# google-research/frame-interpolation

Hardware: NVIDIA H100
Metric: interpolated_frames_per_sec_1080p (higher is better)
Workload: dtype f16x2-split (activations/weights as fp16 hi+lo planes; fp32 accumulate)

## Files before the change

### frame_interpolation_b200/csrc/film_common.cuh

```cuda
#pragma once
#include <cuda_bf16.h>
#include <cuda_fp16.h>
#include <cuda_runtime.h>
#include <stdint.h>

namespace film {

#ifdef FILM_SPLIT_FP16
typedef __half sp_t;
#define FILM_SPLIT_NAME "fp16x2"
#else
typedef __nv_bfloat16 sp_t;
#define FILM_SPLIT_NAME "bf16x2"
#endif

constexpr float kLeaky = 0.2f;

struct ActView {
  sp_t* hi;
  sp_t* lo;
  int B, H, W, C;
};

__device__ __forceinline__ float sp_to_float(sp_t v) {
#ifdef FILM_SPLIT_FP16
  return __half2float(v);
#else
  return __bfloat162float(v);
#endif
}
__device__ __forceinline__ sp_t float_to_sp(float v) {
#ifdef FILM_SPLIT_FP16
  return __float2half_rn(v);
#else
  return __float2bfloat16_rn(v);
#endif
}

__device__ __forceinline__ void split2(float x, sp_t& hi, sp_t& lo) {
  hi = float_to_sp(x);
  lo = float_to_sp(x - sp_to_float(hi));
}

#ifndef FILM_SPLIT_FP16
__device__ __forceinline__ void split_pack2(float a, float b, uint32_t& hi, uint32_t& lo) {
  const __nv_bfloat162 h2 = __floats2bfloat162_rn(a, b);
  hi = *reinterpret_cast<const uint32_t*>(&h2);
  const float ra = a - __uint_as_float(hi << 16);
  const float rb = b - __uint_as_float(hi & 0xffff0000u);
  const __nv_bfloat162 l2 = __floats2bfloat162_rn(ra, rb);
  lo = *reinterpret_cast<const uint32_t*>(&l2);
}
__device__ __forceinline__ void split_pack2_generic(float a, float b, uint32_t& hi, uint32_t& lo) {
#else
__device__ __forceinline__ void split_pack2(float a, float b, uint32_t& hi, uint32_t& lo) {
  asm("cvt.rn.satfinite.f16x2.f32 %0, %1, %2;" : "=r"(hi) : "f"(b), "f"(a));
  const float2 hf = __half22float2(*reinterpret_cast<const __half2*>(&hi));
  asm("cvt.rn.satfinite.f16x2.f32 %0, %1, %2;" : "=r"(lo) : "f"(b - hf.y), "f"(a - hf.x));
}
__device__ __forceinline__ void split_pack2_generic(float a, float b, uint32_t& hi, uint32_t& lo) {
#endif
  sp_t ah, al, bh, bl;
  split2(a, ah, al);
  split2(b, bh, bl);
  hi = (uint32_t)(*reinterpret_cast<unsigned short*>(&ah)) |
       ((uint32_t)(*reinterpret_cast<unsigned short*>(&bh)) << 16);
  lo = (uint32_t)(*reinterpret_cast<unsigned short*>(&al)) |
       ((uint32_t)(*reinterpret_cast<unsigned short*>(&bl)) << 16);
}

__device__ __forceinline__ float sp_bits_to_float(uint32_t bits16) {
#ifdef FILM_SPLIT_FP16
  unsigned short s = (unsigned short)bits16;
  return __half2float(*reinterpret_cast<__half*>(&s));
#else
  return __uint_as_float(bits16 << 16);
#endif
}

__device__ __forceinline__ void unpack8(const uint4& h, const uint4& l, float* v) {
  const uint32_t hw[4] = {h.x, h.y, h.z, h.w};
  const uint32_t lw[4] = {l.x, l.y, l.z, l.w};
#pragma unroll
  for (int i = 0; i < 4; ++i) {
#ifndef FILM_SPLIT_FP16
    v[2 * i] = __uint_as_float(hw[i] << 16) + __uint_as_float(lw[i] << 16);
    v[2 * i + 1] = __uint_as_float(hw[i] & 0xffff0000u) + __uint_as_float(lw[i] & 0xffff0000u);
#else
    const float2 hf = __half22float2(*reinterpret_cast<const __half2*>(&hw[i]));
    const float2 lf = __half22float2(*reinterpret_cast<const __half2*>(&lw[i]));
    v[2 * i] = hf.x + lf.x;
    v[2 * i + 1] = hf.y + lf.y;
#endif
  }
}

__device__ __forceinline__ void pack8(const float* v, uint4& h, uint4& l) {
  split_pack2(v[0], v[1], h.x, l.x);
  split_pack2(v[2], v[3], h.y, l.y);
  split_pack2(v[4], v[5], h.z, l.z);
  split_pack2(v[6], v[7], h.w, l.w);
}

__device__ __forceinline__ void st256(void* p, const uint4& a, const uint4& b) {
  uint4* q = reinterpret_cast<uint4*>(p);
  q[0] = a;
  q[1] = b;
}
__device__ __forceinline__ void ld256_nc(const void* p, uint4& a, uint4& b) {
  const uint4* q = reinterpret_cast<const uint4*>(p);
  a = __ldg(q);
  b = __ldg(q + 1);
}
__device__ __forceinline__ void pack_store16(const float* v, sp_t* hi_dst, sp_t* lo_dst) {
  uint4 h0, l0, h1, l1;
  pack8(v, h0, l0);
  pack8(v + 8, h1, l1);
  st256(hi_dst, h0, h1);
  st256(lo_dst, l0, l1);
}
__device__ __forceinline__ uint32_t pack2_hi(float a, float b) {
#ifdef FILM_SPLIT_FP16
  uint32_t hi;
  asm("cvt.rn.satfinite.f16x2.f32 %0, %1, %2;" : "=r"(hi) : "f"(b), "f"(a));
  return hi;
#else
  const __nv_bfloat162 h2 = __floats2bfloat162_rn(a, b);
  return *reinterpret_cast<const uint32_t*>(&h2);
#endif
}
__device__ __forceinline__ void pack_store16_hi(const float* v, sp_t* hi_dst) {
  uint4 h0, h1;
  h0.x = pack2_hi(v[0], v[1]);   h0.y = pack2_hi(v[2], v[3]);   h0.z = pack2_hi(v[4], v[5]);   h0.w = pack2_hi(v[6], v[7]);
  h1.x = pack2_hi(v[8], v[9]);   h1.y = pack2_hi(v[10], v[11]); h1.z = pack2_hi(v[12], v[13]); h1.w = pack2_hi(v[14], v[15]);
  st256(hi_dst, h0, h1);
}
__device__ __forceinline__ void unpack8_hi(const uint4& h, float* v) {
  const uint32_t hw[4] = {h.x, h.y, h.z, h.w};
#pragma unroll
  for (int i = 0; i < 4; ++i) {
#ifndef FILM_SPLIT_FP16
    v[2 * i] = __uint_as_float(hw[i] << 16);
    v[2 * i + 1] = __uint_as_float(hw[i] & 0xffff0000u);
#else
    const float2 hf = __half22float2(*reinterpret_cast<const __half2*>(&hw[i]));
    v[2 * i] = hf.x;
    v[2 * i + 1] = hf.y;
#endif
  }
}
__device__ __forceinline__ void load_unpack16_hi(const sp_t* hi_src, float* v) {
  uint4 h0, h1;
  ld256_nc(hi_src, h0, h1);
  unpack8_hi(h0, v);
  unpack8_hi(h1, v + 8);
}
__device__ __forceinline__ void load_unpack16(const sp_t* hi_src, const sp_t* lo_src, float* v) {
  uint4 h0, h1, l0, l1;
  ld256_nc(hi_src, h0, h1);
  ld256_nc(lo_src, l0, l1);
  unpack8(h0, l0, v);
  unpack8(h1, l1, v + 8);
}

__device__ __forceinline__ float leaky(float x) { return x >= 0.f ? x : x * kLeaky; }

}
```

### frame_interpolation_b200/csrc/film_conv3x3_tc.cu

```cuda
#include <cuda.h>
#include <cuda_runtime.h>
#include <stdint.h>

#include <type_traits>

#include "film_conv.h"
#include "film_tc_ptx.cuh"

namespace film {
namespace {
using namespace tc;

constexpr int kConsumers = 256;
constexpr int kThreads = kConsumers + 128;
__host__ __device__ constexpr int a_plane_bytes(int kc, int th, int tw) { return (th + 2) * tw * kc * 2; }
__host__ __device__ constexpr int a_stage_bytes(int kc, int th, int tw) { return 2 * a_plane_bytes(kc, th, tw); }
constexpr int kHaloW = 10;
__host__ __device__ constexpr int halo_box_bytes(int kc, int th) { return (th + 2) * kHaloW * kc * 2; }
__host__ __device__ constexpr int halo_plane_bytes(int kc, int th) { return (halo_box_bytes(kc, th) + 1023) & ~1023; }
__host__ __device__ constexpr int a_stage_bytes_h(int kc, int th, int tw, int halo, int planes = 2) {
  return planes * (halo ? halo_plane_bytes(kc, th) : a_plane_bytes(kc, th, tw));
}
constexpr int kMaxRing = 8;
constexpr int kSmemLimit = 227 * 1024;
constexpr int kBarBytes = 8 * (4 * kMaxRing + 4);
constexpr int kFixedBytes = kBarBytes + 16 + 512 * 4  + 64  + 1024  + 64;
constexpr int kHeadW3 = 64 * 32 * 4, kHeadMisc = 512;
constexpr int kHeadBytes = kHeadW3 + kHeadMisc;
constexpr int kPxnStageWg = 64 * 64 * 2;
constexpr int kPxnStageBytes = 2 * kPxnStageWg;
inline int epi_scratch_bytes(int epi_mode, int pxn) { return epi_mode == 3 ? kHeadBytes : pxn ? kPxnStageBytes : 0; }

__host__ __device__ inline int w_tap_bytes(int bn, int kc, int planes = 2) { return bn * kc * 2 * planes; }

template <int BN, int KC, bool kPartial, bool kHalo, bool kOne, bool kRes, bool kPxN = false>
__global__ void __launch_bounds__(kThreads, 1) k_conv3x3_tc(const ConvProblem* __restrict__ prob) {
  static_assert(!kPxN || (BN == 64 && KC == 64), "pixels on N: Cout = 64 (one M = 64 weight tile), 64-channel chunks");
  extern __shared__ uint8_t smem_raw[];
  constexpr bool one = kOne;
  const int planes = one ? 1 : 2;
  constexpr int kWPlane = BN * KC * 2;
  const int kWTap = kWPlane * planes;
  const int kTileH = prob->tile_h, kTileW = prob->tile_w;
  constexpr int kHaloTileH = kPxN ? 32 : 16;
  constexpr int kHaloBox = halo_box_bytes(KC, kHaloTileH), kHaloPlane = halo_plane_bytes(KC, kHaloTileH);
  constexpr bool halo = kHalo;
  const int kAPlane = halo ? kHaloPlane : a_plane_bytes(KC, kTileH, kTileW);
  const int kAStage = planes * kAPlane;
  const int kRowStep = kTileW * KC * 2;
  constexpr bool kFused = BN <= 128 && !kPxN;
  constexpr int kAccRegs = kPxN ? 64 : (kFused ? 2 * BN : BN) / 2;
  constexpr int kWgPx = kPxN ? 128 : 64;

  const int NA = prob->v2_na, NW = prob->v2_nw;
  const bool resident = prob->v2_resident != 0;
  const int nsrc = prob->nsrc;
  const int tiles_x = prob->tiles_x, tiles_per_img = prob->tiles_y * prob->tiles_x;
  const int cout = prob->cout;
  const int n_nt = (cout + BN - 1) / BN;
  const int ntiles = prob->B * tiles_per_img * n_nt;
  constexpr int kStageTaps = kHalo ? 9 : 3;
  constexpr bool kPacked = kPartial && kPxN;
  const int part_lo = prob->v2_part_lo, part_hi = prob->v2_part_hi;
  int nab = 0;
  for (int s = 0; s < nsrc; ++s) nab += prob->src[s].nchunk * (kHalo ? 1 : 3);
  const int nkb = nab * kStageTaps - (kPacked ? (part_hi - part_lo) * (kStageTaps - kStageTaps / 3) : 0);

  const FastDiv div_nt(n_nt, ntiles), div_img(tiles_per_img, ntiles), div_tx(tiles_x, ntiles);
  const bool pair = prob->pair != 0;
  const int rank = pair ? (int)cluster_ctarank() : 0;
  const int nsp = prob->B * tiles_per_img;
  const int nwork = pair ? ((nsp + 1) / 2) * n_nt : ntiles;
  const int w_first = pair ? (int)blockIdx.x >> 1 : (int)blockIdx.x, w_step = pair ? (int)gridDim.x >> 1 : (int)gridDim.x;
  auto decode = [&](int work, int& sp, int& nti) {
    div_nt.divmod(work, sp, nti);
    if (pair) sp = 2 * sp + rank;
  };

  const uint32_t raw = smem_u32(smem_raw);
  const uint32_t base = (raw + 1023u) & ~1023u;
  uint8_t* gen_base = smem_raw + (base - raw);
  const uint32_t a_base = base;
  const uint32_t w_base = a_base + (uint32_t)NA * kAStage;
  const uint32_t w_bytes = resident ? (uint32_t)nkb * kWTap : (uint32_t)NW * kWTap;
  const uint32_t tail = w_base + w_bytes;
  const uint32_t tail_off = (uint32_t)NA * kAStage + w_bytes;
  float* bias_smem = reinterpret_cast<float*>(gen_base + tail_off + kBarBytes + 16);
  int* src_tab = reinterpret_cast<int*>(gen_base + tail_off + kBarBytes + 16 + 512 * 4);

  const int warp = threadIdx.x >> 5, lane = threadIdx.x & 31;

  if (warp == 8 && lane == 0) {
    for (int s = 0; s < kMaxRing; ++s) {
      mbar_init(tail + 8u * s, 1);
      mbar_init(tail + 8u * (kMaxRing + s), 2);
      mbar_init(tail + 8u * (2 * kMaxRing + s), 1);
      mbar_init(tail + 8u * (3 * kMaxRing + s), pair ? 4 : 2);
    }
    for (int s = 0; s < kMaxSrc; ++s) {
      src_tab[2 * s] = s < nsrc ? prob->src[s].nchunk : 0;
      src_tab[2 * s + 1] = s < nsrc ? prob->src[s].c_off : 0;
      src_tab[2 * kMaxSrc + s] = s < nsrc ? prob->src[s].bswap : 0;
    }
    asm volatile("fence.mbarrier_init.release.cluster;" ::: "memory");
  }
  if (warp < 8)
    for (int i = threadIdx.x; i < n_nt * BN; i += kConsumers) bias_smem[i] = (i < cout) ? prob->bias[i] : 0.f;
  __syncthreads();
  if (pair) cluster_sync_all();
  auto leave = [&]() {
    if (pair) cluster_sync_all();
  };

  if (warp >= 8) {
    regs_dec<40>();
    if (warp > 8) {
      leave();
      return;
    }
    const CUtensorMap* tm_w_hi = &prob->tm_w_hi;
    const CUtensorMap* tm_w_lo = &prob->tm_w_lo;
    if (resident && elect_one()) {
      mbar_expect_tx(tail + 8u * (2 * kMaxRing), (uint32_t)nkb * kWTap);
      for (int kb = 0; kb < nkb; ++kb) {
        tma_load_2d(w_base + kb * kWTap, tm_w_hi, tail + 8u * (2 * kMaxRing), kb * KC, 0);
        if (!one) tma_load_2d(w_base + kb * kWTap + kWPlane, tm_w_lo, tail + 8u * (2 * kMaxRing), kb * KC, 0);
      }
    }
    __syncwarp();
    RingPos ra, rw;
    for (int tile = w_first; tile < nwork; tile += w_step) {
      int sp, nti, b, rem, ty, tx;
      decode(tile, sp, nti);
      div_img.divmod(sp, b, rem);
      div_tx.divmod(rem, ty, tx);
      const int n0 = nti * BN, y0 = ty * kTileH, x0 = tx * kTileW;
      {
        const int nt = tile + w_step;
        int next_sp, nnt;
        decode(nt < nwork ? nt : 0, next_sp, nnt);
        if (nt < nwork && next_sp != sp && next_sp < nsp && elect_one()) {
          int nb, nrem, nty, ntx;
          div_img.divmod(next_sp, nb, nrem);
          div_tx.divmod(nrem, nty, ntx);
          const int ny0 = nty * kTileH, nx0 = ntx * kTileW;
          for (int s = 0; s < nsrc; ++s)
            for (int ch = 0; ch < src_tab[2 * s]; ++ch) {
              const int cc = src_tab[2 * s + 1] + ch * KC;
              tma_prefetch_4d(&prob->tm_a_hi[s], cc, nx0 - 1, ny0 - 1, nb);
              if (!one) tma_prefetch_4d(&prob->tm_a_lo[s], cc, nx0 - 1, ny0 - 1, nb);
              if (!halo) {
                tma_prefetch_4d(&prob->tm_a_hi[s], cc, nx0 + 1, ny0 - 1, nb);
                if (!one) tma_prefetch_4d(&prob->tm_a_lo[s], cc, nx0 + 1, ny0 - 1, nb);
              }
            }
        }
        __syncwarp();
      }
      int kb = 0, ab = 0;
      for (int s = 0; s < nsrc; ++s) {
        const int nchunk = src_tab[2 * s], c_off = src_tab[2 * s + 1];
        const int bs = src_tab[2 * kMaxSrc + s] ? prob->B - 1 - b : b;
        const CUtensorMap* tm_hi = &prob->tm_a_hi[s];
        const CUtensorMap* tm_lo = &prob->tm_a_lo[s];
        for (int ch = 0; ch < nchunk; ++ch) {
          const int nst = halo ? 1 : 3;
          for (int dx = 0; dx < nst; ++dx, ++ab) {
            const int st = ra.stage;
            mbar_wait(tail + 8u * (kMaxRing + st), ra.phase ^ 1u);
            if (elect_one()) {
              const uint32_t sa = a_base + st * kAStage, bar = tail + 8u * st;
              mbar_expect_tx(bar, halo ? (uint32_t)(planes * kHaloBox) : (uint32_t)kAStage);
              tma_load_4d(sa, tm_hi, bar, c_off + ch * KC, x0 + dx - 1, y0 - 1, bs);
              if (!one) tma_load_4d(sa + kAPlane, tm_lo, bar, c_off + ch * KC, x0 + dx - 1, y0 - 1, bs);
            }
            __syncwarp();
            ra.advance(NA);
            if (!resident) {
              const bool packed = kPacked && ab >= part_lo && ab < part_hi;
              const int nblk = packed ? kStageTaps / 3 : kStageTaps;
              for (int t = 0; t < nblk; ++t, ++kb) {
                const int ws = rw.stage;
                mbar_wait(tail + 8u * (3 * kMaxRing + ws), rw.phase ^ 1u);
                if (elect_one()) {
                  const uint32_t sw = w_base + ws * kWTap, bar = tail + 8u * (2 * kMaxRing + ws);
                  mbar_expect_tx(bar, kWTap);
                  if (pair) {
                    const uint32_t hoff = (uint32_t)(rank * (kWPlane / 2));
                    tma_load_2d_mc(sw + hoff, &prob->tm_w_hi_half, bar, kb * KC, n0 + rank * (BN / 2), 3);
                    if (!one) tma_load_2d_mc(sw + kWPlane + hoff, &prob->tm_w_lo_half, bar, kb * KC, n0 + rank * (BN / 2), 3);
                  } else {
                    tma_load_2d(sw, tm_w_hi, bar, kb * KC, n0);
                    if (!one) tma_load_2d(sw + kWPlane, tm_w_lo, bar, kb * KC, n0);
                  }
                }
                __syncwarp();
                rw.advance(NW);
              }
            }
          }
        }
      }
    }
    leave();
    return;
  }

  regs_inc<232>();
  const int wg = warp >> 2;
  const int q = lane & 3;
  const int H = prob->H, W = prob->W, out_H = prob->out_H, out_W = prob->out_W, out_C = prob->out_C;
  const int out_c_off = prob->out_c_off, act = prob->act;
  sp_t* const out_hi = prob->out_hi;
  sp_t* const out_lo = prob->out_lo;
  sp_t* const pool_hi = prob->pool_hi;
  sp_t* const pool_lo = prob->pool_lo;
  const int pool_C = prob->pool_C;
  const bool do_pool = pool_hi != nullptr;
  const bool lo_skip = prob->out_lo_skip != 0;
  const bool rgb = prob->epi_mode == 2;
  const float* const head_w = prob->head_w4;
  float* const rgb_out = prob->head_v;
  const int crop_y = prob->crop_y, crop_x = prob->crop_x, crop_h = prob->crop_h, crop_w = prob->crop_w;
  const int64_t crop_pitch = prob->crop_pitch;
  const bool fhead = prob->epi_mode == 3;
  constexpr int kHid = BN <= 64 ? BN / 2 : 1;
  float* const w3s = reinterpret_cast<float*>(reinterpret_cast<uint8_t*>(src_tab) + 64);
  float* const hmisc = w3s + kHeadW3 / 4;
  if (fhead) {
    if constexpr (BN <= 64) {
      for (int i = threadIdx.x; i < BN * kHid; i += kConsumers) w3s[i] = prob->head_w3[i];
      for (int i = threadIdx.x; i < kHid; i += kConsumers) hmisc[i] = prob->head_b3[i];
      for (int i = threadIdx.x; i < 2 * kHid; i += kConsumers) hmisc[kHid + i] = prob->head_w4[i];
      if (threadIdx.x < 2) hmisc[3 * kHid + threadIdx.x] = prob->head_b4[threadIdx.x];
    }
    asm volatile("bar.sync 1, %0;" ::"r"(kConsumers) : "memory");
  }
  const float* const head_vup = prob->head_vup;
  float* const head_res = prob->head_res;
  float* const head_vout = prob->head_v;

  if (resident) mbar_wait(tail + 8u * (2 * kMaxRing), 0);
  const bool is_leader = (threadIdx.x & 127) == 0;
  const uint32_t w_empty_peer = pair ? map_to_cta(tail + 8u * (3 * kMaxRing), (uint32_t)(rank ^ 1)) : 0u;
  auto release_w = [&](int slot) {
    mbar_arrive(tail + 8u * (3 * kMaxRing + slot));
    if (pair) mbar_arrive_cluster(w_empty_peer + 8u * slot);
  };
  {
    constexpr int kWTapC = kWPlane * (kOne ? 1 : 2);
    constexpr uint32_t kPx = KC * 2;
    const uint32_t a_row0 = kHalo ? (uint32_t)(wg * (kWgPx / 8) * kHaloW) * kPx : (uint32_t)(wg * kWgPx) * kPx;
    const uint32_t sbo = kHalo ? kHaloW * kPx : 8 * kPx;
    RingPos ra, rw;
    float acc[kAccRegs];
    for (int tile = w_first; tile < nwork; tile += w_step) {
      int kb = 0;
      int rel_a = -1, rel_w = -1;
      auto retire = [&](int next_a, int next_w) {
        wgmma_commit();
        wgmma_wait<1>();
        if (is_leader) {
          if (rel_a >= 0) mbar_arrive(tail + 8u * (kMaxRing + rel_a));
          if (rel_w >= 0) release_w(rel_w);
        }
        rel_a = next_a;
        rel_w = next_w;
      };
      auto stage = [&](auto ksteps_c, auto tpb_c) {
        constexpr int kSteps = decltype(ksteps_c)::value, kTpb = decltype(tpb_c)::value;
        constexpr int kBlocks = kStageTaps / kTpb;
        const int st = ra.stage;
        mbar_wait(tail + 8u * st, ra.phase);
        const uint32_t sa = a_base + st * kAStage + a_row0;
        const uint32_t lo_off = (uint32_t)(kHalo ? kHaloPlane : kAPlane);
        if constexpr (kRes) {
          const uint64_t a0 = make_desc_sbo<KC>(sa, sbo);
          const uint64_t lo_delta = (uint64_t)(lo_off >> 4);
          const uint64_t row_delta = (uint64_t)(kRowStep >> 4);
          const uint64_t w0 = make_desc_kc<KC>(w_base + kb * kWTapC);
          const uint32_t first = (kb == 0) ? 0u : 1u;
          wgmma_fence();
#pragma unroll
          for (int t = 0; t < kStageTaps; ++t) {
            const uint64_t a_hi = a0 + (kHalo ? (uint64_t)((((t % 3) * kHaloW + t / 3) * kPx) >> 4) : (uint64_t)t * row_delta);
            const uint64_t a_lo = a_hi + lo_delta;
            const uint64_t w_hi = w0 + (uint64_t)(((t / kTpb) * kWTapC + (t % kTpb) * kSteps * 32) >> 4);
            const uint64_t w_lo = w_hi + (uint64_t)(kWPlane >> 4);
#pragma unroll
            for (int k = 0; k < kSteps; ++k) {
              const uint64_t adv = (uint64_t)(k * 32 >> 4);
              const uint32_t accf = (t == 0 && k == 0) ? first : 1u;
              if constexpr (kPxN) {
                wgmma<128>(acc, w_hi + adv, a_hi + adv, accf);
                if constexpr (!kOne) {
                  wgmma<128>(acc, w_lo + adv, a_hi + adv, 1u);
                  wgmma<128>(acc, w_hi + adv, a_lo + adv, 1u);
                }
              } else if constexpr (kOne) {
                wgmma<BN>(acc, a_hi + adv, w_hi + adv, accf);
              } else if constexpr (kFused) {
                wgmma<BN>(acc, a_hi + adv, w_hi + adv, accf);
                wgmma<BN>(acc + BN / 2, a_hi + adv, w_lo + adv, accf);
                wgmma<BN>(acc, a_lo + adv, w_hi + adv, 1u);
              } else {
                wgmma<BN>(acc, a_lo + adv, w_hi + adv, accf);
                wgmma<BN>(acc, a_hi + adv, w_lo + adv, 1u);
                wgmma<BN>(acc, a_hi + adv, w_hi + adv, 1u);
              }
            }
          }
          retire(st, -1);
          kb += kBlocks;
        } else {
          for (int blk = 0; blk < kBlocks; ++blk, ++kb) {
            uint32_t sw;
            int ws = -1;
            if (resident) {
              sw = w_base + kb * kWTap;
            } else {
              ws = rw.stage;
              mbar_wait(tail + 8u * (2 * kMaxRing + ws), rw.phase);
              sw = w_base + ws * kWTap;
            }
            const uint32_t first = (kb == 0) ? 0u : 1u;
            wgmma_fence();
#pragma unroll
            for (int u = 0; u < kTpb; ++u) {
              const int t = blk * kTpb + u;
              const uint32_t off = kHalo ? (uint32_t)((t % 3) * kHaloW + t / 3) * kPx : (uint32_t)(t * kRowStep);
              const uint64_t a_hi = make_desc_sbo<KC>(sa + off, sbo);
              const uint64_t a_lo = make_desc_sbo<KC>(sa + lo_off + off, sbo);
              const uint64_t wk = (uint64_t)((u * kSteps * 32) >> 4);
              const uint64_t w_hi = make_desc_kc<KC>(sw) + wk, w_lo = make_desc_kc<KC>(sw + kWPlane) + wk;
#pragma unroll
              for (int k = 0; k < kSteps; ++k) {
                const uint64_t adv = (uint64_t)(k * 32 >> 4);
                const uint32_t accf = (u == 0 && k == 0) ? first : 1u;
                if constexpr (kPxN) {
                  wgmma<128>(acc, w_hi + adv, a_hi + adv, accf);
                  if constexpr (!kOne) {
                    wgmma<128>(acc, w_lo + adv, a_hi + adv, 1u);
                    wgmma<128>(acc, w_hi + adv, a_lo + adv, 1u);
                  }
                } else if constexpr (kOne) {
                  wgmma<BN>(acc, a_hi + adv, w_hi + adv, accf);
                } else if constexpr (kFused) {
                  wgmma<BN>(acc, a_hi + adv, w_hi + adv, accf);
                  wgmma<BN>(acc + BN / 2, a_hi + adv, w_lo + adv, accf);
                  wgmma<BN>(acc, a_lo + adv, w_hi + adv, 1u);
                } else {
                  wgmma<BN>(acc, a_lo + adv, w_hi + adv, accf);
                  wgmma<BN>(acc, a_hi + adv, w_lo + adv, 1u);
                  wgmma<BN>(acc, a_hi + adv, w_hi + adv, 1u);
                }
              }
            }
            retire(blk == kBlocks - 1 ? st : -1, ws);
            if (!resident) rw.advance(NW);
          }
        }
        ra.advance(NA);
      };
      using Full = std::integral_constant<int, KC / 16>;
      using One = std::integral_constant<int, 1>;
      if constexpr (kPartial) {
        for (int ab = 0; ab < part_lo; ++ab) stage(Full{}, One{});
        for (int ab = part_lo; ab < part_hi; ++ab) stage(One{}, std::integral_constant<int, kPacked ? 3 : 1>{});
        for (int ab = part_hi; ab < nab; ++ab) stage(Full{}, One{});
      } else {
        for (int ab = 0; ab < nab; ++ab) stage(Full{}, One{});
      }
      wgmma_wait<0>();
      if (is_leader) {
        if (rel_a >= 0) mbar_arrive(tail + 8u * (kMaxRing + rel_a));
        if (rel_w >= 0) release_w(rel_w);
      }
      acc_fence<kAccRegs>(acc);

      int sp, nti, b, rem, ty, tx;
      decode(tile, sp, nti);
      div_img.divmod(sp, b, rem);
      div_tx.divmod(rem, ty, tx);
      const int n0 = nti * BN;
      const bool live = sp < nsp;
      if constexpr (kPxN) {
        const int c0 = 16 * (warp & 3) + (lane >> 2);
        const float bias0 = bias_smem[c0], bias1 = bias_smem[c0 + 8];
#pragma unroll
        for (int i = 0; i < kAccRegs; ++i) {
          const float f = acc[i] + ((i & 2) ? bias1 : bias0);
          acc[i] = act ? leaky(f) : f;
        }
        const int y_wg = ty * kTileH + 16 * wg, x_t = tx * kTileW;
        if (do_pool) {
          const int px = x_t + 2 * q;
#pragma unroll
          for (int j = 0; j < 16; j += 2) {
            const int py = y_wg + j;
            const bool ok = live && (py >> 1) < (out_H >> 1) && (px >> 1) < (out_W >> 1) && !(lane & 4);
            const int64_t ppix = ((int64_t)b * (out_H >> 1) + (py >> 1)) * (out_W >> 1) + (px >> 1);
#pragma unroll
            for (int h = 0; h < 2; ++h) {
              const int i = 4 * j + 2 * h;
              const float v = ((acc[i] + acc[i + 1]) + (acc[i + 4] + acc[i + 5])) * 0.25f;
              const float vn = __shfl_xor_sync(0xffffffffu, v, 4);
              if (ok) {
                uint32_t hi, lo;
                split_pack2(v, vn, hi, lo);
                *reinterpret_cast<uint32_t*>(pool_hi + ppix * pool_C + c0 + 8 * h) = hi;
                *reinterpret_cast<uint32_t*>(pool_lo + ppix * pool_C + c0 + 8 * h) = lo;
              }
            }
          }
        }
        uint8_t* const stg = reinterpret_cast<uint8_t*>(src_tab) + 64 + wg * kPxnStageWg;
        const uint32_t stg_u = smem_u32(stg);
        const int t128 = threadIdx.x & 127;
        auto wg_sync = [&]() { asm volatile("bar.sync %0, 128;" ::"r"(2 + wg) : "memory"); };
        for (int pl = 0; pl < (lo_skip ? 1 : 2); ++pl) {
          sp_t* const dst = pl ? out_lo : out_hi;
#pragma unroll
          for (int half = 0; half < 2; ++half) {
            wg_sync();
#pragma unroll
            for (int jj = 0; jj < 8; jj += 2) {
              uint32_t r[4];
#pragma unroll
              for (int m = 0; m < 4; ++m) {
                const int i = 4 * (8 * half + jj + (m >> 1)) + 2 * (m & 1);
                if (pl) {
                  uint32_t hi;
                  split_pack2(acc[i], acc[i + 1], hi, r[m]);
                } else {
                  r[m] = pack2_hi(acc[i], acc[i + 1]);
                }
              }
              const int p = 8 * (jj + (lane >> 4)) + (lane & 7), ch = 2 * (warp & 3) + ((lane >> 3) & 1);
              stmatrix_x4_trans(stg_u + p * 128 + ((ch ^ (p & 7)) << 4), r[0], r[1], r[2], r[3]);
            }
            wg_sync();
#pragma unroll
            for (int k = 0; k < 4; ++k) {
              const int idx = 128 * k + t128, p = idx >> 3, ch = idx & 7;
              const int py = y_wg + 8 * half + (p >> 3), px = x_t + (p & 7);
              if (live && py < H && px < W) {
                const uint4 v = *reinterpret_cast<const uint4*>(stg + p * 128 + ((ch ^ (p & 7)) << 4));
                const int64_t opix = ((int64_t)b * out_H + py) * out_W + px;
                *reinterpret_cast<uint4*>(dst + opix * out_C + out_c_off + 8 * ch) = v;
              }
            }
          }
        }
        continue;
      }
      auto value = [&](int h, int j, int e) {
        const int i = 4 * j + 2 * h + e;
        return (kFused && !kOne) ? acc[i] + acc[(i + BN / 2) % kAccRegs] : acc[i];
      };
#pragma unroll
      for (int h = 0; h < 2 && (fhead || rgb); ++h) {
        const int r = wg * 64 + (warp & 3) * 16 + (lane >> 2) + 8 * h;
        const int py = ty * kTileH + r / kTileW, px = tx * kTileW + r % kTileW;
        const bool valid = live && (py < H) && (px < W);
        const int64_t opix = ((int64_t)b * out_H + py) * out_W + px;
        if (fhead) {
          if constexpr (BN <= 64) {
            float hp[kHid];
#pragma unroll
            for (int hh = 0; hh < kHid; ++hh) hp[hh] = 0.f;
#pragma unroll
            for (int j = 0; j < BN / 8; ++j)
#pragma unroll
              for (int e = 0; e < 2; ++e) {
                const int c = 8 * j + 2 * q + e;
                const float x = value(h, j, e) + bias_smem[n0 + c];
                const float f = act ? leaky(x) : x;
                const float4* wr = reinterpret_cast<const float4*>(w3s + c * kHid);
#pragma unroll
                for (int h4 = 0; h4 < kHid / 4; ++h4) {
                  const float4 wv = wr[h4];
                  hp[4 * h4] = fmaf(f, wv.x, hp[4 * h4]);
                  hp[4 * h4 + 1] = fmaf(f, wv.y, hp[4 * h4 + 1]);
                  hp[4 * h4 + 2] = fmaf(f, wv.z, hp[4 * h4 + 2]);
                  hp[4 * h4 + 3] = fmaf(f, wv.w, hp[4 * h4 + 3]);
                }
              }
#pragma unroll
            for (int hh = 0; hh < kHid; ++hh) {
              hp[hh] += __shfl_xor_sync(0xffffffffu, hp[hh], 1);
              hp[hh] += __shfl_xor_sync(0xffffffffu, hp[hh], 2);
            }
            if (q == 0 && valid) {
              float f0 = hmisc[3 * kHid], f1 = hmisc[3 * kHid + 1];
#pragma unroll
              for (int hh = 0; hh < kHid; ++hh) {
                const float x = leaky(hp[hh] + hmisc[hh]);
                f0 = fmaf(x, hmisc[kHid + 2 * hh], f0);
                f1 = fmaf(x, hmisc[kHid + 2 * hh + 1], f1);
              }
              float2 res = make_float2(f0, f1), tot = res;
              if (head_vup) {
                const float2 u = reinterpret_cast<const float2*>(head_vup)[opix];
                tot.x += u.x;
                tot.y += u.y;
              }
              reinterpret_cast<float2*>(head_res)[opix] = res;
              reinterpret_cast<float2*>(head_vout)[opix] = tot;
            }
          }
        } else if (rgb) {
          float r0 = 0.f, r1 = 0.f, r2 = 0.f;
#pragma unroll
          for (int j = 0; j < BN / 8; ++j)
#pragma unroll
            for (int e = 0; e < 2; ++e) {
              const int c = n0 + 8 * j + 2 * q + e;
              float f = value(h, j, e) + bias_smem[c];
              if (act) f = leaky(f);
              r0 = fmaf(f, __ldg(head_w + 3 * c), r0);
              r1 = fmaf(f, __ldg(head_w + 3 * c + 1), r1);
              r2 = fmaf(f, __ldg(head_w + 3 * c + 2), r2);
            }
#pragma unroll
          for (int m = 1; m <= 2; m <<= 1) {
            r0 += __shfl_xor_sync(0xffffffffu, r0, m);
            r1 += __shfl_xor_sync(0xffffffffu, r1, m);
            r2 += __shfl_xor_sync(0xffffffffu, r2, m);
          }
          const int oy = py - crop_y, ox = px - crop_x;
          if (q == 0 && valid && oy >= 0 && oy < crop_h && ox >= 0 && ox < crop_w) {
            float* o = rgb_out + (int64_t)oy * crop_pitch + (int64_t)ox * 3;
            o[0] = r0 + __ldg(prob->head_b4);
            o[1] = r1 + __ldg(prob->head_b4 + 1);
            o[2] = r2 + __ldg(prob->head_b4 + 2);
          }
        }
      }
      if (!fhead && !rgb) {
        bool valid[2];
        int64_t opix[2];
#pragma unroll
        for (int h = 0; h < 2; ++h) {
          const int r = wg * 64 + (warp & 3) * 16 + (lane >> 2) + 8 * h;
          const int py = ty * kTileH + r / kTileW, px = tx * kTileW + r % kTileW;
          valid[h] = live && (py < H) && (px < W);
          opix[h] = ((int64_t)b * out_H + py) * out_W + px;
        }
        const int r0 = wg * 64 + (warp & 3) * 16 + (lane >> 2);
        const int py0 = ty * kTileH + r0 / kTileW, px0 = tx * kTileW + r0 % kTileW;
        const bool pool_ok = live && (py0 >> 1) < (out_H >> 1) && (px0 >> 1) < (out_W >> 1) && !(lane & 4);
        const int64_t ppix = ((int64_t)b * (out_H >> 1) + (py0 >> 1)) * (out_W >> 1) + (px0 >> 1);
#pragma unroll
        for (int j = 0; j < BN / 8; ++j) {
          const int c = 8 * j + 2 * q;
          if (n0 + c >= cout) break;
          float a[2][2];
#pragma unroll
          for (int h = 0; h < 2; ++h) {
            float f0 = value(h, j, 0) + bias_smem[n0 + c], f1 = value(h, j, 1) + bias_smem[n0 + c + 1];
            if (act) {
              f0 = leaky(f0);
              f1 = leaky(f1);
            }
            if (valid[h]) {
              sp_t* oh = out_hi + opix[h] * out_C + out_c_off + n0;
              if (lo_skip) {
                *reinterpret_cast<uint32_t*>(oh + c) = pack2_hi(f0, f1);
              } else {
                sp_t* ol = out_lo + opix[h] * out_C + out_c_off + n0;
                uint32_t hi, lo;
                split_pack2(f0, f1, hi, lo);
                *reinterpret_cast<uint32_t*>(oh + c) = hi;
                *reinterpret_cast<uint32_t*>(ol + c) = lo;
              }
            }
            if (do_pool) {
              a[h][0] = f0 + __shfl_xor_sync(0xffffffffu, f0, 4);
              a[h][1] = f1 + __shfl_xor_sync(0xffffffffu, f1, 4);
            }
          }
          if (do_pool && pool_ok) {
            uint32_t hi, lo;
            split_pack2((a[0][0] + a[1][0]) * 0.25f, (a[0][1] + a[1][1]) * 0.25f, hi, lo);
            *reinterpret_cast<uint32_t*>(pool_hi + ppix * pool_C + n0 + c) = hi;
            *reinterpret_cast<uint32_t*>(pool_lo + ppix * pool_C + n0 + c) = lo;
          }
        }
      }
    }
  }
  leave();
}

int smem_bytes_for(const ConvProblem& h, int bn) {
  const int nkb = h.ktot / h.kchunk;
  const int planes = h.passes == 1 ? 1 : 2;
  const int w = h.v2_resident ? nkb * w_tap_bytes(bn, h.kchunk, planes) : h.v2_nw * w_tap_bytes(bn, h.kchunk, planes);
  return h.v2_na * a_stage_bytes_h(h.kchunk, h.tile_h, h.tile_w, h.halo, planes) + w + kFixedBytes +
         epi_scratch_bytes(h.epi_mode, h.pxn);
}

}

int conv_tc_block_n(int cout);

namespace {
bool ring_depths(int kc, int tile_h, int tile_w, int halo, int planes, int bn, int cout, int ktot, int epi_mode, int pxn,
                 int& resident, int& na, int& nw) {
  const int wtap = w_tap_bytes(bn, kc, planes);
  const int w_all = (ktot / kc) * wtap;
  const int kLimit = kSmemLimit - epi_scratch_bytes(epi_mode, pxn);
  const int kAStage = a_stage_bytes_h(kc, tile_h, tile_w, halo, planes);
  if (cout <= bn && w_all + 2 * kAStage + kFixedBytes <= kLimit) {
    resident = 1;
    const int n = (kLimit - kFixedBytes - w_all) / kAStage;
    const int n_max = halo ? 3 : 6;
    na = n > n_max ? n_max : n;
    nw = 1;
    return true;
  }
  resident = 0;
  na = halo ? 2 : (bn >= 128 ? 2 : 3);
  int n = (kLimit - kFixedBytes - na * kAStage) / wtap;
  if (n < 2 && na > 2) {
    na = 2;
    n = (kLimit - kFixedBytes - na * kAStage) / wtap;
  }
  nw = n > kMaxRing ? kMaxRing : n;
  return nw >= 2;
}
}

void conv3x3_tc_pick_tile(int H, int W, int B, int cout, int kc, int passes, int ktot, int epi_mode, int num_sms,
                          int& tile_h, int& tile_w) {
  static const int cand[3][2] = {{16, 8}, {8, 16}, {4, 32}};
  const int bn = conv_tc_block_n(cout);
  const int n_nt = (cout + bn - 1) / bn;
  double best = 1e30;
  tile_h = 16;
  tile_w = 8;
  for (auto& c : cand) {
    int res, na, nw;
    if (!ring_depths(kc, c[0], c[1], 0, passes == 1 ? 1 : 2, bn, cout, ktot, epi_mode, 0, res, na, nw)) continue;
    const long tiles = (long)B * ((H + c[0] - 1) / c[0]) * ((W + c[1] - 1) / c[1]) * n_nt;
    const long waves = (tiles + num_sms - 1) / num_sms;
    const double cost = (double)waves * (c[0] + 2.0) / c[0] * (1.0 + 1e-3 * (c[1] / 8));
    if (cost < best) {
      best = cost;
      tile_h = c[0];
      tile_w = c[1];
    }
  }
}

bool conv3x3_tc_plan(ConvProblem& h, int num_sms) {
  const int bn = h.bn;
  const int planes = h.passes == 1 ? 1 : 2;
  const int wtap = w_tap_bytes(bn, h.kchunk, planes);
  const int w_all = (h.ktot / h.kchunk) * wtap;
  const bool can_resident = h.cout <= bn;
  const int kLimit = kSmemLimit - epi_scratch_bytes(h.epi_mode, h.pxn);
  if (h.halo && (h.tile_h != (h.pxn ? 32 : 16) || h.tile_w != 8 ||
                 (can_resident && w_all + 2 * a_stage_bytes_h(h.kchunk, h.tile_h, h.tile_w, 0, planes) + kFixedBytes <= kLimit &&
                  w_all + 2 * a_stage_bytes_h(h.kchunk, h.tile_h, h.tile_w, 1, planes) + kFixedBytes > kLimit)))
    h.halo = 0;
  bool ok = ring_depths(h.kchunk, h.tile_h, h.tile_w, h.halo, planes, bn, h.cout, h.ktot, h.epi_mode, h.pxn,
                        h.v2_resident, h.v2_na, h.v2_nw);
  if (!ok && h.halo) {
    h.halo = 0;
    ok = ring_depths(h.kchunk, h.tile_h, h.tile_w, 0, planes, bn, h.cout, h.ktot, h.epi_mode, h.pxn, h.v2_resident,
                     h.v2_na, h.v2_nw);
  }
  const int nsp = h.B * h.tiles_y * h.tiles_x, n_nt = (h.cout + bn - 1) / bn;
  if (h.pair) {
    const int nwork = (nsp + 1) / 2 * n_nt, nclu = num_sms / 2;
    h.v2_grid = 2 * (nwork < nclu ? nwork : nclu);
  } else {
    h.v2_grid = nsp * n_nt < num_sms ? nsp * n_nt : num_sms;
  }
  return ok;
}

template <int BN, int KC, bool kPxN = false>
struct Variants {
  static constexpr void (*kFn[16])(const ConvProblem*) = {
      k_conv3x3_tc<BN, KC, false, false, false, false, kPxN>, k_conv3x3_tc<BN, KC, false, false, false, true, kPxN>,
      k_conv3x3_tc<BN, KC, false, false, true, false, kPxN>,  k_conv3x3_tc<BN, KC, false, false, true, true, kPxN>,
      k_conv3x3_tc<BN, KC, false, true, false, false, kPxN>,  k_conv3x3_tc<BN, KC, false, true, false, true, kPxN>,
      k_conv3x3_tc<BN, KC, false, true, true, false, kPxN>,   k_conv3x3_tc<BN, KC, false, true, true, true, kPxN>,
      k_conv3x3_tc<BN, KC, true, false, false, false, kPxN>,  k_conv3x3_tc<BN, KC, true, false, false, true, kPxN>,
      k_conv3x3_tc<BN, KC, true, false, true, false, kPxN>,   k_conv3x3_tc<BN, KC, true, false, true, true, kPxN>,
      k_conv3x3_tc<BN, KC, true, true, false, false, kPxN>,   k_conv3x3_tc<BN, KC, true, true, false, true, kPxN>,
      k_conv3x3_tc<BN, KC, true, true, true, false, kPxN>,    k_conv3x3_tc<BN, KC, true, true, true, true, kPxN>};
  static cudaError_t configure() {
    for (auto fn : kFn) {
      const cudaError_t e = cudaFuncSetAttribute(fn, cudaFuncAttributeMaxDynamicSharedMemorySize, kSmemLimit);
      if (e != cudaSuccess) return e;
    }
    return cudaSuccess;
  }
  static cudaError_t launch(const ConvProblem* d_prob, const ConvProblem& h, cudaStream_t st) {
    if (h.v2_na < 2 || (!h.v2_resident && h.v2_nw < 2)) return cudaErrorInvalidValue;
    if (kPxN && (h.pair || h.tile_h != 32 || h.tile_w != 8 || h.epi_mode != 0)) return cudaErrorInvalidValue;
    const bool partial = h.v2_part_hi > h.v2_part_lo;
    const int idx = (partial ? 8 : 0) | (h.halo ? 4 : 0) | (h.passes == 1 ? 2 : 0) | (h.v2_resident && h.straight ? 1 : 0);
    if (!h.pair) {
      kFn[idx]<<<h.v2_grid, kThreads, smem_bytes_for(h, BN), st>>>(d_prob);
      return cudaGetLastError();
    }
    cudaLaunchConfig_t cfg = {};
    cudaLaunchAttribute attr[1];
    attr[0].id = cudaLaunchAttributeClusterDimension;
    attr[0].val.clusterDim.x = 2;
    attr[0].val.clusterDim.y = 1;
    attr[0].val.clusterDim.z = 1;
    cfg.gridDim = dim3(h.v2_grid);
    cfg.blockDim = dim3(kThreads);
    cfg.dynamicSmemBytes = smem_bytes_for(h, BN);
    cfg.stream = st;
    cfg.attrs = attr;
    cfg.numAttrs = 1;
    return cudaLaunchKernelEx(&cfg, kFn[idx], d_prob);
  }
};

cudaError_t conv3x3_tc_configure() {
  cudaError_t e;
#define FILM_CFG(BN, KC)                        \
  e = Variants<BN, KC>::configure();            \
  if (e != cudaSuccess) return e;
  FILM_CFG(32, 64) FILM_CFG(64, 64) FILM_CFG(128, 64) FILM_CFG(256, 64) FILM_CFG(32, 32) FILM_CFG(64, 32)
#undef FILM_CFG
  e = Variants<64, 64, true>::configure();
  if (e != cudaSuccess) return e;
  return cudaSuccess;
}

cudaError_t launch_conv3x3_tc(const ConvProblem* d_prob, const ConvProblem& h, cudaStream_t st) {
  const int bn = h.bn;
  if (h.kchunk == 32) {
    if (bn == 32) return Variants<32, 32>::launch(d_prob, h, st);
    if (bn == 64) return Variants<64, 32>::launch(d_prob, h, st);
    return cudaErrorInvalidValue;
  }
  switch (bn) {
    case 256: return Variants<256, 64>::launch(d_prob, h, st);
    case 128: return Variants<128, 64>::launch(d_prob, h, st);
    case 64: return h.pxn ? Variants<64, 64, true>::launch(d_prob, h, st) : Variants<64, 64>::launch(d_prob, h, st);
    default: return Variants<32, 64>::launch(d_prob, h, st);
  }
}

}
```

### frame_interpolation_b200/csrc/film_conv_tc.cu

```cuda
#include <cuda.h>
#include <cuda_runtime.h>
#include <cstdio>
#include <stdint.h>

#include "film_conv.h"
#include "film_tc_ptx.cuh"

namespace film {

namespace {
using namespace tc;

constexpr int kConsumers = 256;
constexpr int kNumThreads = kConsumers + 128;
template <int BN, int KC>
struct TcCfg {
  static constexpr int kABytes = kTileM * KC * 2;
  static constexpr int kWBytes = BN * KC * 2;
  static constexpr int kStageBytes = 2 * kABytes + 2 * kWBytes;
  static constexpr int kStages = (BN == 256) ? 2 : (BN == 128) ? 3 : 2;
  static constexpr bool kFused = BN <= 128;
  static constexpr int kAccRegs = (kFused ? 2 * BN : BN) / 2;
  static constexpr int kSmemBytes = kStages * kStageBytes + 1024  + 256 + BN * 4 + BN * 8 + 16;
};

template <int BN, int KC>
__global__ void __launch_bounds__(kNumThreads, 1) k_conv_tc(const ConvProblem* __restrict__ prob_base) {
  using Cfg = TcCfg<BN, KC>;
  const ConvProblem* __restrict__ prob = prob_base + blockIdx.z;
  constexpr int kABytes = Cfg::kABytes;
  extern __shared__ uint8_t smem_raw[];

  const uint32_t raw = smem_u32(smem_raw);
  const uint32_t base = (raw + 1023u) & ~1023u;
  uint8_t* gen_base = smem_raw + (base - raw);
  const uint32_t bar_base = base + Cfg::kStages * Cfg::kStageBytes;
  auto full_bar = [&](int s) { return bar_base + 8u * s; };
  auto empty_bar = [&](int s) { return bar_base + 8u * (Cfg::kStages + s); };
  float* bias_smem = reinterpret_cast<float*>(gen_base + Cfg::kStages * Cfg::kStageBytes + 256);
  float* w4_smem = bias_smem + BN;

  const int warp = threadIdx.x >> 5;
  const int lane = threadIdx.x & 31;

  const int nsrc = prob->nsrc, ntaps = prob->ntaps, cout = prob->cout, epi_mode = prob->epi_mode;
  const bool one = prob->passes == 1;
  const int tile_h = prob->tile_h, tile_w = prob->tile_w, tiles_x = prob->tiles_x, tiles_y = prob->tiles_y;

  int tile = blockIdx.x;
  const int tx = tile % tiles_x;
  tile /= tiles_x;
  const int ty = tile % tiles_y;
  const int b = tile / tiles_y;
  const int y0 = ty * tile_h, x0 = tx * tile_w;
  const int n0 = blockIdx.y * BN;

  int nkb = 0;
  for (int s = 0; s < nsrc; ++s) nkb += prob->src[s].nchunk * ntaps;

  if (warp == 8 && lane == 0) {
    for (int s = 0; s < Cfg::kStages; ++s) {
      mbar_init(full_bar(s), 1);
      mbar_init(empty_bar(s), 2);
    }
    asm volatile("fence.mbarrier_init.release.cluster;" ::: "memory");
  }
  if (warp < 8) {
    for (int i = threadIdx.x; i < BN; i += kConsumers) bias_smem[i] = (n0 + i < cout) ? prob->bias[n0 + i] : 0.f;
    if (epi_mode == 1) {
      for (int i = threadIdx.x; i < 2 * BN; i += kConsumers) w4_smem[i] = (i < 2 * cout) ? prob->head_w4[i] : 0.f;
      if (threadIdx.x < 2) w4_smem[2 * BN + threadIdx.x] = prob->head_b4[threadIdx.x];
    }
  }
  __syncthreads();

  if (warp >= 8) {
    regs_dec<40>();
    if (warp > 8) return;
    const CUtensorMap* tm_w_hi = &prob->tm_w_hi;
    const CUtensorMap* tm_w_lo = &prob->tm_w_lo;
    int kb = 0;
    for (int s = 0; s < nsrc; ++s) {
      const int nchunk = prob->src[s].nchunk, c_off = prob->src[s].c_off;
      const int bs = prob->src[s].bswap ? prob->B - 1 - b : b;
      const CUtensorMap* tm_hi = &prob->tm_a_hi[s];
      const CUtensorMap* tm_lo = &prob->tm_a_lo[s];
      for (int ch = 0; ch < nchunk; ++ch) {
        for (int t = 0; t < ntaps; ++t, ++kb) {
          const int stage = kb % Cfg::kStages;
          const uint32_t phase = (uint32_t)(kb / Cfg::kStages) & 1u;
          const int xx = x0 + prob->tap_dx[t], yy = y0 + prob->tap_dy[t];
          mbar_wait(empty_bar(stage), phase ^ 1u);
          if (elect_one()) {
            const uint32_t sa = base + stage * Cfg::kStageBytes;
            mbar_expect_tx(full_bar(stage), one ? (uint32_t)(kABytes + Cfg::kWBytes) : (uint32_t)Cfg::kStageBytes);
            const int cc = c_off + ch * KC;
            tma_load_4d(sa, tm_hi, full_bar(stage), cc, xx, yy, bs);
            tma_load_2d(sa + 2 * kABytes, tm_w_hi, full_bar(stage), kb * KC, n0);
            if (!one) {
              tma_load_4d(sa + kABytes, tm_lo, full_bar(stage), cc, xx, yy, bs);
              tma_load_2d(sa + 2 * kABytes + Cfg::kWBytes, tm_w_lo, full_bar(stage), kb * KC, n0);
            }
          }
          __syncwarp();
        }
      }
    }
    return;
  }

  regs_inc<232>();
  const int wg = warp >> 2;
  const uint32_t a_row0 = (uint32_t)(wg * 64 * KC * 2);
  float acc[Cfg::kAccRegs];
#pragma unroll
  for (int i = 0; i < Cfg::kAccRegs; ++i) acc[i] = 0.f;
  int prev_stage = -1;
  for (int kb = 0; kb < nkb; ++kb) {
    const int stage = kb % Cfg::kStages;
    const uint32_t phase = (uint32_t)(kb / Cfg::kStages) & 1u;
    mbar_wait(full_bar(stage), phase);
    const uint32_t sa = base + stage * Cfg::kStageBytes;
    const uint64_t a_hi = make_desc_kc<KC>(sa + a_row0), a_lo = make_desc_kc<KC>(sa + kABytes + a_row0);
    const uint64_t w_hi = make_desc_kc<KC>(sa + 2 * kABytes), w_lo = make_desc_kc<KC>(sa + 2 * kABytes + Cfg::kWBytes);
    const uint32_t first = kb == 0 ? 0u : 1u;
    wgmma_fence();
#pragma unroll
    for (int k = 0; k < KC / 16; ++k) {
      const uint64_t adv = (uint64_t)(k * 32 >> 4);
      if (one) {
        wgmma<BN>(acc, a_hi + adv, w_hi + adv, k == 0 ? first : 1u);
      } else if constexpr (Cfg::kFused) {
        wgmma<BN>(acc, a_hi + adv, w_hi + adv, k == 0 ? first : 1u);
        wgmma<BN>(acc + BN / 2, a_hi + adv, w_lo + adv, k == 0 ? first : 1u);
        wgmma<BN>(acc, a_lo + adv, w_hi + adv, 1u);
      } else {
        wgmma<BN>(acc, a_lo + adv, w_hi + adv, k == 0 ? first : 1u);
        wgmma<BN>(acc, a_hi + adv, w_lo + adv, 1u);
        wgmma<BN>(acc, a_hi + adv, w_hi + adv, 1u);
      }
    }
    wgmma_commit();
    wgmma_wait<1>();
    if (prev_stage >= 0 && (threadIdx.x & 127) == 0) mbar_arrive(empty_bar(prev_stage));
    prev_stage = stage;
  }
  wgmma_wait<0>();
  acc_fence<Cfg::kAccRegs>(acc);

  const bool fused3 = Cfg::kFused && !one;
  auto value = [&](int h, int j, int e) {
    const int i = 4 * j + 2 * h + e;
    return fused3 ? acc[i] + acc[(i + BN / 2) % Cfg::kAccRegs] : acc[i];
  };
  const int q = lane & 3;
  const float* head_vup = prob->head_vup;
  float* head_res = prob->head_res;
  float* head_v = prob->head_v;
#pragma unroll
  for (int h = 0; h < 2; ++h) {
    const int r = wg * 64 + (warp & 3) * 16 + (lane >> 2) + 8 * h;
    const int py = y0 + r / tile_w, px = x0 + r % tile_w;
    const bool valid = (py < prob->H) && (px < prob->W);
    const int64_t opix = ((int64_t)b * prob->out_H + ((int64_t)py * prob->out_sy + prob->out_oy)) * prob->out_W +
                         ((int64_t)px * prob->out_sx + prob->out_ox);
    if (epi_mode == 1) {
      float r0 = 0.f, r1 = 0.f;
#pragma unroll
      for (int j = 0; j < BN / 8; ++j)
#pragma unroll
        for (int e = 0; e < 2; ++e) {
          const int c = 8 * j + 2 * q + e;
          const float hdn = leaky(value(h, j, e) + bias_smem[c]);
          r0 = fmaf(hdn, w4_smem[c * 2], r0);
          r1 = fmaf(hdn, w4_smem[c * 2 + 1], r1);
        }
      r0 += __shfl_xor_sync(0xffffffffu, r0, 1);
      r1 += __shfl_xor_sync(0xffffffffu, r1, 1);
      r0 += __shfl_xor_sync(0xffffffffu, r0, 2);
      r1 += __shfl_xor_sync(0xffffffffu, r1, 2);
      if (valid && q == 0) {
        float2 res = make_float2(r0 + w4_smem[2 * BN], r1 + w4_smem[2 * BN + 1]);
        float2 tot = res;
        if (head_vup) {
          const float2 u = reinterpret_cast<const float2*>(head_vup)[opix];
          tot.x += u.x;
          tot.y += u.y;
        }
        reinterpret_cast<float2*>(head_res)[opix] = res;
        reinterpret_cast<float2*>(head_v)[opix] = tot;
      }
    } else if (valid) {
      const int act = prob->act;
      sp_t* oh = prob->out_hi + opix * prob->out_C + prob->out_c_off + n0;
      sp_t* ol = prob->out_lo + opix * prob->out_C + prob->out_c_off + n0;
      const bool lo_skip = prob->out_lo_skip != 0;
#pragma unroll
      for (int j = 0; j < BN / 8; ++j) {
        const int c = 8 * j + 2 * q;
        if (n0 + c >= cout) break;
        float f0 = value(h, j, 0) + bias_smem[c], f1 = value(h, j, 1) + bias_smem[c + 1];
        if (act) {
          f0 = leaky(f0);
          f1 = leaky(f1);
        }
        uint32_t hi, lo;
        if (lo_skip) {
          *reinterpret_cast<uint32_t*>(oh + c) = pack2_hi(f0, f1);
        } else {
          split_pack2(f0, f1, hi, lo);
          *reinterpret_cast<uint32_t*>(oh + c) = hi;
          *reinterpret_cast<uint32_t*>(ol + c) = lo;
        }
      }
    }
  }
}

template <int BN, int KC>
cudaError_t launch_bn(const ConvProblem* d_prob, const ConvProblem& h, cudaStream_t st) {
  dim3 grid(h.B * h.tiles_y * h.tiles_x, (h.cout + BN - 1) / BN, h.group > 1 ? h.group : 1);
  k_conv_tc<BN, KC><<<grid, kNumThreads, TcCfg<BN, KC>::kSmemBytes, st>>>(d_prob);
  return cudaGetLastError();
}

}

int conv_tc_block_n(int cout) { return cout >= 256 ? 256 : cout >= 128 ? 128 : cout >= 64 ? 64 : 32; }

cudaError_t conv_tc_configure() {
  cudaError_t e;
#define FILM_CFG(BN, KC)                                                                         \
  e = cudaFuncSetAttribute(k_conv_tc<BN, KC>, cudaFuncAttributeMaxDynamicSharedMemorySize,      \
                           TcCfg<BN, KC>::kSmemBytes);                                           \
  if (e != cudaSuccess) return e;
  FILM_CFG(32, 64) FILM_CFG(64, 64) FILM_CFG(128, 64) FILM_CFG(256, 64) FILM_CFG(32, 32) FILM_CFG(64, 32)
#undef FILM_CFG
  return cudaSuccess;
}

cudaError_t launch_conv_tc(const ConvProblem* d_prob, const ConvProblem& h, cudaStream_t st) {
  const int bn = h.bn;
  if (h.kchunk == 32) {
    if (bn == 64) return launch_bn<64, 32>(d_prob, h, st);
    if (bn == 32) return launch_bn<32, 32>(d_prob, h, st);
    return cudaErrorInvalidValue;
  }
  switch (bn) {
    case 256: return launch_bn<256, 64>(d_prob, h, st);
    case 128: return launch_bn<128, 64>(d_prob, h, st);
    case 64: return launch_bn<64, 64>(d_prob, h, st);
    default: return launch_bn<32, 64>(d_prob, h, st);
  }
}

}
```

### frame_interpolation_b200/csrc/film_engine.cu

```cuda
#include <cuda.h>
#include <cuda_runtime.h>

#include <algorithm>
#include <cmath>
#include <cstdio>
#include <cstdlib>
#include <cstring>
#include <functional>
#include <map>
#include <memory>
#include <string>
#include <vector>

#include "../../include/film_b200.h"
#include "film_conv.h"
#include "film_kernels.h"
#include "film_pack.h"

namespace film {
int conv_tc_block_n(int cout);

constexpr int kLevels = 7, kFusionLevels = 5, kSpecialized = 3, kSubLevels = 4, kFilters = 64;
static const int kFlowFilters[4] = {32, 64, 128, 256};
static const char* kPredictorNames[4] = {"flow_predictor_0", "flow_predictor_1", "flow_predictor_2",
                                         "flow_predictor_shared"};
static int feat_channels(int l) {
  int c = 0;
  for (int j = 0; j <= (l < kSubLevels - 1 ? l : kSubLevels - 1); ++j) c += kFilters << j;
  return c;
}
static int fusion_filters(int l) { return l < kSpecialized ? (kFilters << l) : (kFilters << kSpecialized); }
static int round_up(int a, int b) { return (a + b - 1) / b * b; }

struct Error {
  int code;
  std::string msg;
};

enum Stage {
  ST_FE_I0_K01 = 0, ST_FE_I0_K23, ST_FE_I0_K45, ST_FE_I0_K67,
  ST_FE_I1, ST_FE_I2, ST_FE_I3P,
  ST_FLOW_L0,
  ST_FUS = ST_FLOW_L0 + kLevels,
  ST_COUNT = ST_FUS + 3 * (kFusionLevels - 1),
  ST_NONE = -1
};
static std::string stage_name(int s) {
  static const char* fe[] = {"fe_i0_k01", "fe_i0_k23", "fe_i0_k45", "fe_i0_k67", "fe_i1", "fe_i2", "fe_i3p"};
  if (s < 0 || s >= ST_COUNT) return "";
  if (s < ST_FLOW_L0) return fe[s];
  if (s < ST_FUS) return "flow_L" + std::to_string(s - ST_FLOW_L0);
  return "fus" + std::to_string((s - ST_FUS) / 3) + "_c" + std::to_string((s - ST_FUS) % 3);
}
static int fe_stage(int image_level, int conv_k) {
  if (image_level == 0) return ST_FE_I0_K01 + conv_k / 2;
  return image_level == 1 ? ST_FE_I1 : image_level == 2 ? ST_FE_I2 : ST_FE_I3P;
}
constexpr uint32_t kDefaultOnepassMask =
    (1u << ST_FE_I0_K23) | (1u << ST_FE_I0_K45) | (1u << ST_FE_I0_K67) |
    (0x1Fu << ST_FLOW_L0) | (0x3Fu << (ST_FUS + 6));

struct Options {
  int conv_impl = 0;
  int use_graph = 1;
  int keep_debug = 0;
  int time_ops = 0;
  int use_lanes = 0;
  int conv3x3_v2 = 1;
  int conv3x3_2cta = 0;
  int conv3x3_halo = 3;
  int conv3x3_pxn = 1;
  int onepass_mask = (int)kDefaultOnepassMask;
  int fe_conv0_tc = 0;
  int fuse_rgb_head = 1;
  int fuse_flow_head = 1;
  int plane_skip = 1;
  int mma_straight = 1;
  int arena_reuse = 1;
  int any_size = 0;
  int tile_overlap = 0;
};

static int as_given(int v) { return v; }
static int as_bool(int v) { return v ? 1 : 0; }
static int clamp_0_2(int v) { return v < 0 ? 0 : (v > 2 ? 2 : v); }
static int non_negative(int v) { return v < 0 ? 0 : v; }
static int stage_bits(int v) { return (int)((uint32_t)v & ((1u << ST_COUNT) - 1u)); }
struct OptionRow {
  const char* name;
  int Options::*field;
  int (*normalise)(int);
  const char* env;
  bool plan_key;
};
static const OptionRow kOptions[] = {
    {"conv_impl", &Options::conv_impl, as_given, nullptr, true},
    {"use_graph", &Options::use_graph, as_given, nullptr, false},
    {"keep_debug", &Options::keep_debug, as_given, nullptr, true},
    {"time_ops", &Options::time_ops, as_given, nullptr, false},
    {"use_lanes", &Options::use_lanes, as_given, nullptr, true},
    {"conv3x3_v2", &Options::conv3x3_v2, as_given, nullptr, true},
    {"conv3x3_2cta", &Options::conv3x3_2cta, as_given, "FILM_2CTA", true},
    {"conv3x3_halo", &Options::conv3x3_halo, as_given, "FILM_HALO", true},
    {"conv3x3_pxn", &Options::conv3x3_pxn, clamp_0_2, nullptr, true},
    {"onepass_mask", &Options::onepass_mask, stage_bits, "FILM_ONEPASS", true},
    {"fe_conv0_tc", &Options::fe_conv0_tc, as_bool, "FILM_FE0_TC", true},
    {"fuse_rgb_head", &Options::fuse_rgb_head, as_bool, "FILM_RGB_FUSE", true},
    {"fuse_flow_head", &Options::fuse_flow_head, clamp_0_2, "FILM_FLOW_HEAD_FUSE", true},
    {"plane_skip", &Options::plane_skip, as_bool, "FILM_PLANE_SKIP", true},
    {"mma_straight", &Options::mma_straight, as_bool, "FILM_STRAIGHT", true},
    {"arena_reuse", &Options::arena_reuse, as_bool, "FILM_ARENA_REUSE", true},
    {"any_size", &Options::any_size, as_bool, nullptr, false},
    {"tile_overlap", &Options::tile_overlap, non_negative, nullptr, false},
};
static const OptionRow& option_row(const char* name) {
  for (const OptionRow& r : kOptions)
    if (!strcmp(r.name, name)) return r;
  throw Error{FILM_ERR_ARG, std::string("unknown option ") + name};
}

#define FILM_CUDA(expr)                                                                       \
  do {                                                                                        \
    cudaError_t e__ = (expr);                                                                 \
    if (e__ != cudaSuccess)                                                                   \
      throw Error{FILM_ERR_CUDA, std::string(#expr) + ": " + cudaGetErrorString(e__)};        \
  } while (0)

struct HostTensor {
  std::vector<int> dims;
  std::vector<float> data;
};
typedef std::map<std::string, HostTensor> WeightMap;

static WeightMap read_weight_file(const char* path) {
  FILE* f = fopen(path, "rb");
  if (!f) throw Error{FILM_ERR_WEIGHTS, std::string("cannot open weight file ") + path};
  WeightMap m;
  auto fail = [&](const char* why) {
    fclose(f);
    throw Error{FILM_ERR_WEIGHTS, std::string(path) + ": " + why};
  };
  char magic[8];
  if (fread(magic, 1, 8, f) != 8 || memcmp(magic, "FILMW1\0\0", 8) != 0) fail("bad magic");
  uint32_t n;
  if (fread(&n, 4, 1, f) != 1) fail("truncated");
  for (uint32_t i = 0; i < n; ++i) {
    uint32_t ln, nd;
    if (fread(&ln, 4, 1, f) != 1 || ln > 4096) fail("bad name length");
    std::string name(ln, '\0');
    if (fread(&name[0], 1, ln, f) != ln) fail("truncated");
    if (fread(&nd, 4, 1, f) != 1 || nd > 8) fail("bad rank");
    HostTensor t;
    size_t cnt = 1;
    for (uint32_t d = 0; d < nd; ++d) {
      uint32_t v;
      if (fread(&v, 4, 1, f) != 1) fail("truncated");
      t.dims.push_back((int)v);
      cnt *= v;
    }
    t.data.resize(cnt);
    if (fread(t.data.data(), 4, cnt, f) != cnt) fail("truncated tensor data");
    m[name] = std::move(t);
  }
  fclose(f);
  return m;
}

static const HostTensor& get_tensor(const WeightMap& m, const std::string& name, std::vector<int> dims) {
  auto it = m.find(name);
  if (it == m.end()) throw Error{FILM_ERR_WEIGHTS, "missing tensor " + name};
  if (it->second.dims != dims) throw Error{FILM_ERR_WEIGHTS, "shape mismatch for " + name};
  return it->second;
}

static uint16_t f32_to_bf16(float f) {
  uint32_t u;
  memcpy(&u, &f, 4);
  if ((u & 0x7fffffffu) > 0x7f800000u) return (uint16_t)((u >> 16) | 0x40);
  u += 0x7fffu + ((u >> 16) & 1u);
  return (uint16_t)(u >> 16);
}
static float bf16_to_f32(uint16_t h) {
  uint32_t u = (uint32_t)h << 16;
  float f;
  memcpy(&f, &u, 4);
  return f;
}
static uint16_t f32_to_sp(float f) {
#ifdef FILM_SPLIT_FP16
  __half h = __float2half_rn(f);
  uint16_t u;
  memcpy(&u, &h, 2);
  return u;
#else
  return f32_to_bf16(f);
#endif
}
static float sp_to_f32(uint16_t h) {
#ifdef FILM_SPLIT_FP16
  __half v;
  memcpy(&v, &h, 2);
  return __half2float(v);
#else
  return bf16_to_f32(h);
#endif
}

struct PackedConv {
  sp_t* w_hi = nullptr;
  sp_t* w_lo = nullptr;
  float* bias = nullptr;
  int cout = 0, ktot = 0, cin_ref = 0;
  int kchunk = kChunk;
  std::vector<int> src_chunks;
  std::vector<int> src_ksteps;
  sp_t* pxn_hi = nullptr;
  sp_t* pxn_lo = nullptr;
  int pxn_ktot = 0;
  int ntaps = 0;
  int tap_dy[kMaxTaps], tap_dx[kMaxTaps];
};

struct TapSpec {
  int dy, dx;
  std::vector<std::pair<int, int>> terms;
};

static PackedConv pack_conv(const HostTensor& kernel, const HostTensor& bias,
                            const std::vector<std::vector<int>>& src_maps,
                            const std::vector<TapSpec>& taps, std::vector<void*>& allocs, int chunk = kChunk) {
  const int kw = kernel.dims[1], cin = kernel.dims[2], cout = kernel.dims[3];
  PackedConv pc;
  pc.cout = cout;
  pc.cin_ref = cin;
  pc.kchunk = chunk;
  pc.ntaps = (int)taps.size();
  for (size_t t = 0; t < taps.size(); ++t) {
    pc.tap_dy[t] = taps[t].dy;
    pc.tap_dx[t] = taps[t].dx;
  }
  int ktot = 0;
  for (auto& sm : src_maps) {
    if (sm.size() % chunk) throw Error{FILM_ERR_WEIGHTS, "source channel map not a multiple of the K chunk"};
    pc.src_chunks.push_back((int)sm.size() / chunk);
    int ks = 1;
    for (size_t i = 0; i < sm.size(); ++i)
      if (sm[i] >= 0) ks = std::max(ks, (int)(i % chunk) / 16 + 1);
    pc.src_ksteps.push_back(ks);
    ktot += (int)sm.size() * (int)taps.size();
  }
  pc.ktot = ktot;
  std::vector<uint16_t> hi((size_t)cout * ktot), lo((size_t)cout * ktot);
  int kbase = 0;
  for (auto& sm : src_maps) {
    const int nchunk = (int)sm.size() / chunk;
    for (int ch = 0; ch < nchunk; ++ch) {
      for (size_t t = 0; t < taps.size(); ++t, kbase += chunk) {
        for (int c = 0; c < chunk; ++c) {
          const int ref = sm[ch * chunk + c];
          for (int n = 0; n < cout; ++n) {
            float w = 0.f;
            if (ref >= 0) {
              if (ref >= cin) throw Error{FILM_ERR_WEIGHTS, "channel map out of range"};
              for (auto& term : taps[t].terms)
                w += kernel.data[(((size_t)term.first * kw + term.second) * cin + ref) * cout + n];
            }
            const uint16_t h = f32_to_sp(w);
            const uint16_t l = f32_to_sp(w - sp_to_f32(h));
            hi[(size_t)n * ktot + kbase + c] = h;
            lo[(size_t)n * ktot + kbase + c] = l;
          }
        }
      }
    }
  }
  auto upload = [&](const std::vector<uint16_t>& v) {
    sp_t* d;
    FILM_CUDA(cudaMalloc(&d, v.size() * 2));
    allocs.push_back(d);
    FILM_CUDA(cudaMemcpy(d, v.data(), v.size() * 2, cudaMemcpyHostToDevice));
    return d;
  };
  pc.w_hi = upload(hi);
  pc.w_lo = upload(lo);
  pc.pxn_hi = pc.w_hi;
  pc.pxn_lo = pc.w_lo;
  pc.pxn_ktot = ktot;
  std::vector<int> packed;
  for (int ks : pc.src_ksteps) packed.push_back(taps.size() == 9 && chunk == kChunk && ks == 1);
  if (std::count(packed.begin(), packed.end(), 1)) {
    pc.pxn_hi = upload(pack_dx_blocks(hi, cout, ktot, chunk, pc.src_chunks, packed, pc.pxn_ktot));
    pc.pxn_lo = upload(pack_dx_blocks(lo, cout, ktot, chunk, pc.src_chunks, packed, pc.pxn_ktot));
  }
  FILM_CUDA(cudaMalloc(&pc.bias, cout * 4));
  allocs.push_back(pc.bias);
  FILM_CUDA(cudaMemcpy(pc.bias, bias.data.data(), cout * 4, cudaMemcpyHostToDevice));
  return pc;
}

static std::vector<TapSpec> taps_3x3() {
  std::vector<TapSpec> t;
  for (int kx = 0; kx < 3; ++kx)
    for (int ky = 0; ky < 3; ++ky) t.push_back({ky - 1, kx - 1, {{ky, kx}}});
  return t;
}
static std::vector<TapSpec> taps_up2x2(int py, int px) {
  std::vector<TapSpec> t;
  for (int dy = 0; dy <= py; ++dy)
    for (int dx = 0; dx <= px; ++dx) {
      TapSpec s{dy, dx, {}};
      for (int fy = 0; fy < 2; ++fy)
        for (int fx = 0; fx < 2; ++fx)
          if ((py + fy) / 2 == dy && (px + fx) / 2 == dx) s.terms.push_back({fy, fx});
      t.push_back(s);
    }
  return t;
}
static std::vector<int> iota_map(int start, int n, int padded) {
  std::vector<int> m(padded, -1);
  for (int i = 0; i < n; ++i) m[i] = start + i;
  return m;
}
static std::vector<int> side_map(int C) {
  std::vector<int> m(kChunk, -1);
  for (int c = 0; c < 3; ++c) m[c] = c;
  for (int c = 0; c < 3; ++c) m[3 + c] = 3 + C + c;
  m[6] = 6 + 2 * C;
  m[7] = 7 + 2 * C;
  m[8] = 8 + 2 * C;
  m[9] = 9 + 2 * C;
  return m;
}

struct Model {
  std::vector<void*> allocs;
  float *conv0_w = nullptr, *conv0_b = nullptr;
  PackedConv fe[8];
  PackedConv fe0_3x3;
  PackedConv flow[4][3];
  PackedConv flow_c3[4];
  float *flow_w3[4], *flow_b3[4], *flow_w4[4], *flow_b4[4];
  PackedConv fus_up[4][4];
  PackedConv fus_up_2x2[4];
  PackedConv fus_c1[4], fus_c2[4];
  float *rgb_w = nullptr, *rgb_b = nullptr;

  float* upload(const HostTensor& t) {
    float* d;
    FILM_CUDA(cudaMalloc(&d, t.data.size() * 4));
    allocs.push_back(d);
    FILM_CUDA(cudaMemcpy(d, t.data.data(), t.data.size() * 4, cudaMemcpyHostToDevice));
    return d;
  }

  void load(const WeightMap& w) {
    const std::string fe_pre = "feat_net/sub_extractor/cfeat_conv_";
    conv0_w = upload(get_tensor(w, fe_pre + "0/kernel", {3, 3, 3, 64}));
    conv0_b = upload(get_tensor(w, fe_pre + "0/bias", {64}));
    {
      HostTensor k0 = get_tensor(w, fe_pre + "0/kernel", {3, 3, 3, 64});
      k0.dims = {1, 1, 27, 64};
      fe[0] = pack_conv(k0, get_tensor(w, fe_pre + "0/bias", {64}), {iota_map(0, 27, 32)},
                        {TapSpec{0, 0, {{0, 0}}}}, allocs, 32);
      fe0_3x3 = pack_conv(get_tensor(w, fe_pre + "0/kernel", {3, 3, 3, 64}), get_tensor(w, fe_pre + "0/bias", {64}),
                          {iota_map(0, 3, 32)}, taps_3x3(), allocs, 32);
    }
    int cin = 64;
    for (int k = 1; k < 8; ++k) {
      const int c = kFilters << (k / 2);
      fe[k] = pack_conv(get_tensor(w, fe_pre + std::to_string(k) + "/kernel", {3, 3, cin, c}),
                        get_tensor(w, fe_pre + std::to_string(k) + "/bias", {c}),
                        {iota_map(0, cin, cin)}, taps_3x3(), allocs);
      cin = c;
    }
    for (int p = 0; p < 4; ++p) {
      const std::string pre = std::string("predict_flow/") + kPredictorNames[p] + "/conv_";
      const int nf = kFlowFilters[p], C = feat_channels(p);
      flow[p][0] = pack_conv(get_tensor(w, pre + "0/kernel", {3, 3, 2 * C, nf}),
                             get_tensor(w, pre + "0/bias", {nf}),
                             {iota_map(0, C, C), iota_map(C, C, C)}, taps_3x3(), allocs);
      const int kc = nf < kChunk ? 32 : kChunk;
      for (int k = 1; k < 3; ++k)
        flow[p][k] = pack_conv(get_tensor(w, pre + std::to_string(k) + "/kernel", {3, 3, nf, nf}),
                               get_tensor(w, pre + std::to_string(k) + "/bias", {nf}),
                               {iota_map(0, nf, round_up(nf, kc))}, taps_3x3(), allocs, kc);
      flow_c3[p] = pack_conv(get_tensor(w, pre + "3/kernel", {1, 1, nf, nf / 2}),
                             get_tensor(w, pre + "3/bias", {nf / 2}), {iota_map(0, nf, round_up(nf, kc))},
                             {TapSpec{0, 0, {{0, 0}}}}, allocs, kc);
      flow_w3[p] = upload(get_tensor(w, pre + "3/kernel", {1, 1, nf, nf / 2}));
      flow_b3[p] = upload(get_tensor(w, pre + "3/bias", {nf / 2}));
      flow_w4[p] = upload(get_tensor(w, pre + "4/kernel", {1, 1, nf / 2, 2}));
      flow_b4[p] = upload(get_tensor(w, pre + "4/bias", {2}));
    }
    for (int i = 0; i < kFusionLevels - 1; ++i) {
      const std::string pre = "fusion/level_" + std::to_string(i) + "/conv_";
      const int nf = fusion_filters(i), C = feat_channels(i);
      const bool from_pyr = (i == kFusionLevels - 2);
      const int Cc = feat_channels(i + 1);
      const int coarse_c = from_pyr ? 2 * (3 + Cc) + 4 : fusion_filters(i + 1);
      const HostTensor& k0 = get_tensor(w, pre + "0/kernel", {2, 2, coarse_c, nf});
      const HostTensor& b0 = get_tensor(w, pre + "0/bias", {nf});
      std::vector<std::vector<int>> up_src;
      if (from_pyr)
        up_src = {iota_map(3, Cc, Cc), iota_map(6 + Cc, Cc, Cc), side_map(Cc)};
      else
        up_src = {iota_map(0, coarse_c, coarse_c)};
      for (int py = 0; py < 2; ++py)
        for (int px = 0; px < 2; ++px)
          fus_up[i][py * 2 + px] = pack_conv(k0, b0, up_src, taps_up2x2(py, px), allocs);
      fus_up_2x2[i] = pack_conv(k0, b0, up_src, {{0, 0, {{0, 0}}}, {0, 1, {{0, 1}}}, {1, 0, {{1, 0}}}, {1, 1, {{1, 1}}}},
                                allocs);
      const int a_c = 2 * (3 + C) + 4;
      fus_c1[i] = pack_conv(get_tensor(w, pre + "1/kernel", {3, 3, a_c + nf, nf}),
                            get_tensor(w, pre + "1/bias", {nf}),
                            {iota_map(3, C, C), iota_map(6 + C, C, C), side_map(C),
                             iota_map(a_c, nf, round_up(nf, kChunk))},
// ... 523 lines not shown
      P.add_op(1, "flow_warp@L" + std::to_string(l), [=](cudaStream_t st) {
        return launch_flow_warp(vprev, hc, wc, f->hi, f->lo, hh, ww, C, vu, warped->hi, warped->lo, hi_only, st);
      }, 0, wbytes);
      P.warp_bytes += wbytes;
      second = warped;
      for (int d = 0; d < 2; ++d) {
        P.debug["flow_warped" + std::to_string(d) + "/" + std::to_string(l)] =
            DebugTensor{true, warped->hi + (int64_t)d * hh * ww * C, warped->lo + (int64_t)d * hh * ww * C, (int64_t)hh * ww,
                        C, 0, C};
        P.debug["flow_vup" + std::to_string(d) + "/" + std::to_string(l)] =
            DebugTensor{false, vup + (int64_t)d * hh * ww * 2, nullptr, (int64_t)hh * ww, 2, 0, 2};
      }
    }
    const int cpad = round_up(nf, nf < kChunk ? 32 : kChunk);
    SplitBuf* c0 = P.split(2, hh, ww, cpad);
    SplitBuf* c1 = P.split(2, hh, ww, cpad);
    SplitBuf* c2 = P.split(2, hh, ww, cpad);
    const std::string lt = "@L" + std::to_string(l);
    std::vector<SrcRef> flow_src(2);
    flow_src[0].buf = feat[l];
    flow_src[0].c_off = 0;
    flow_src[1].buf = second ? second : feat[l];
    flow_src[1].c_off = 0;
    flow_src[1].bswap = second ? 0 : 1;
    add_conv(P, "flow_conv0" + lt, 9.0 * 2 * C * nf, M.flow[p][0], flow_src, 1, c0, 0, ST_FLOW_L0 + l, ST_FLOW_L0 + l);
    add_conv(P, "flow_conv1" + lt, 9.0 * nf * nf, M.flow[p][1], {{c0, 0}}, 1, c1, 0, ST_FLOW_L0 + l, ST_FLOW_L0 + l);
    const bool fuse_head = opt.conv_impl == 0 && opt.conv3x3_v2 && opt.fuse_flow_head && nf <= (opt.fuse_flow_head >= 2 ? 64 : 32);
    if (fuse_head) {
      const size_t ci = add_conv(P, "flow_conv2+head" + lt, 9.0 * nf * nf + 1.0 * nf * (nf / 2) + (nf / 2) * 2.0, M.flow[p][2],
                                 {{c1, 0}}, 1, nullptr, 0, ST_FLOW_L0 + l, ST_NONE, 1, 1, 0, 0, nullptr, false, 3);
      ConvProblem& hp = P.h_probs[ci];
      if (hp.bn != nf) throw Error{FILM_ERR_UNSUPPORTED, "flow-head epilogue expects one N tile on the single-CTA kernel"};
      hp.head_w3 = M.flow_w3[p];
      hp.head_b3 = M.flow_b3[p];
      hp.head_w4 = M.flow_w4[p];
      hp.head_b4 = M.flow_b4[p];
      hp.head_vup = vup;
      hp.head_res = res[l];
      hp.head_v = v[l];
    } else {
      add_conv(P, "flow_conv2" + lt, 9.0 * nf * nf, M.flow[p][2], {{c1, 0}}, 1, c2, 0, ST_FLOW_L0 + l, ST_NONE);
    }
    if (fuse_head) {
    } else if (opt.conv_impl == 1) {
      const float *w3 = M.flow_w3[p], *b3 = M.flow_b3[p], *w4 = M.flow_w4[p], *b4 = M.flow_b4[p];
      float *rr = res[l], *vv = v[l];
      const float* vu = vup;
      const int npix = 2 * hh * ww;
      P.add_op(2, "flow_head" + lt, [=](cudaStream_t st) {
        return launch_flow_head(c2->hi, c2->lo, c2->C, nf, npix, w3, b3, w4, b4, vu, rr, vv, st);
      });
    } else {
      const size_t ci = add_conv(P, "flow_head" + lt, 1.0 * nf * (nf / 2) + (nf / 2) * 2.0, M.flow_c3[p], {{c2, 0}}, 1,
                                 nullptr, 0, ST_NONE, ST_NONE);
      ConvProblem& hp = P.h_probs[ci];
      hp.epi_mode = 1;
      hp.head_w4 = M.flow_w4[p];
      hp.head_b4 = M.flow_b4[p];
      hp.head_vup = vup;
      hp.head_res = res[l];
      hp.head_v = v[l];
    }
    P.release(second);
    P.release(vup);
    P.release(c0);
    P.release(c1);
    P.release(c2);
    if (l >= kFusionLevels) P.release(feat[l]);
    const int64_t np = (int64_t)hh * ww;
    P.debug["flow_fwd/" + std::to_string(l)] = DebugTensor{false, v[l], nullptr, np, 2, 0, 2};
    P.debug["flow_bwd/" + std::to_string(l)] = DebugTensor{false, v[l] + np * 2, nullptr, np, 2, 0, 2};
    P.debug["res_fwd/" + std::to_string(l)] = DebugTensor{false, res[l], nullptr, np, 2, 0, 2};
    P.debug["res_bwd/" + std::to_string(l)] = DebugTensor{false, res[l] + np * 2, nullptr, np, 2, 0, 2};
  }

  SplitBuf* wf[kFusionLevels];
  SplitBuf* side[kFusionLevels];
  for (int l = 0; l < kFusionLevels; ++l) {
    const int C = feat_channels(l), hh = Hs[l], ww = Ws[l];
    wf[l] = P.split(2, hh, ww, C);
    side[l] = P.split(1, hh, ww, kChunk, true);
    const float* vv = v[l];
    const float* im = img[l];
    const SplitBuf *f = feat[l], *o = wf[l], *sd = side[l];
    const int cons = l == kFusionLevels - 1 ? ST_FUS + 3 * (l - 1) : ST_FUS + 3 * l + 1;
    const bool hi_only = P.hi_only(cons);
    const double wbytes = 2.0 * hh * ww * (double)C * (hi_only ? 4.0 : 8.0);
    P.add_op(1, "fusion_warp@L" + std::to_string(l), [=](cudaStream_t st) {
      return launch_fusion_warp(vv, f->hi, f->lo, hh, ww, C, o->hi, o->lo, hi_only, st);
    }, 0, wbytes);
    P.add_op(2, "fusion_side@L" + std::to_string(l), [=](cudaStream_t st) {
      return launch_fusion_side(vv, im, hh, ww, sd->hi, sd->lo, sd->C, st);
    });
    P.warp_bytes += wbytes + 2.0 * hh * ww * 3.0 * 8.0;
    P.release(feat[l]);
    P.debug["aligned_side/" + std::to_string(l)] =
        DebugTensor{true, sd->hi, sd->lo, (int64_t)hh * ww, sd->C, 0, 10};
    for (int k = 0; k < 2; ++k)
      P.debug["warped" + std::to_string(k) + "/" + std::to_string(l)] =
          DebugTensor{true, o->hi + (int64_t)k * hh * ww * C, o->lo + (int64_t)k * hh * ww * C, (int64_t)hh * ww, C, 0, C};
  }
  auto batch_view = [&](const SplitBuf* b, int k) {
    P.bufs.emplace_back(new SplitBuf(*b));
    SplitBuf* s = P.bufs.back().get();
    s->B = 1;
    s->hi = b->hi + (int64_t)k * b->H * b->W * b->C;
    s->lo = b->lo + (int64_t)k * b->H * b->W * b->C;
    return (const SplitBuf*)s;
  };

  const SplitBuf* net = nullptr;
  for (int i = kFusionLevels - 2; i >= 0; --i) {
    const int nf = fusion_filters(i), hh = Hs[i], ww = Ws[i];
    const int cpad = round_up(nf, kChunk);
    SplitBuf* up = P.split(1, hh, ww, cpad);
    std::vector<SrcRef> up_src;
    if (i == kFusionLevels - 2)
      up_src = {{batch_view(wf[i + 1], 0), 0}, {batch_view(wf[i + 1], 1), 0}, {side[i + 1], 0}};
    else
      up_src = {{net, 0}};
    if (hh != 2 * Hs[i + 1] || ww != 2 * Ws[i + 1]) {
      const bool hi_only = P.hi_only(ST_FUS + 3 * i);
      std::vector<std::pair<const SplitBuf*, SplitBuf*>> jobs;
      if (i == kFusionLevels - 2) {
        jobs.push_back({wf[i + 1], P.split(2, hh, ww, wf[i + 1]->C)});
        jobs.push_back({side[i + 1], P.split(1, hh, ww, side[i + 1]->C)});
        up_src = {{batch_view(jobs[0].second, 0), 0}, {batch_view(jobs[0].second, 1), 0}, {jobs[1].second, 0}};
      } else {
        jobs.push_back({net, P.split(1, hh, ww, net->C)});
        up_src = {{jobs[0].second, 0}};
      }
      double rbytes = 0;
      for (auto& j : jobs) rbytes += (double)j.second->pixels() * j.second->C * (hi_only ? 4.0 : 8.0);
      P.add_op(2, "fusion_resize@L" + std::to_string(i), [jobs, hi_only](cudaStream_t st) {
        for (auto& j : jobs) {
          const SplitBuf *s = j.first, *d = j.second;
          const cudaError_t e = launch_resize_nearest(s->hi, s->lo, s->C, 0, s->B, s->H, s->W, d->hi, d->lo, d->C, 0, d->H,
                                                      d->W, d->C, hi_only, st);
          if (e != cudaSuccess) return e;
        }
        return cudaSuccess;
      }, 0, rbytes);
      for (size_t k = 0; k < jobs.size(); ++k) {
        const SplitBuf* d = jobs[k].second;
        P.debug["out:" + P.ops.back().name + (k ? ":side" : "")] = DebugTensor{true, d->hi, d->lo, d->pixels(), d->C, 0, d->C};
      }
      add_conv(P, "fusion_up@L" + std::to_string(i), 4.0 * M.fus_up_2x2[i].cin_ref * nf, M.fus_up_2x2[i], up_src, 0, up, 0,
               ST_FUS + 3 * i, ST_FUS + 3 * i + 1);
      for (auto& j : jobs) P.release(j.second);
    } else if (opt.conv_impl == 0) {
      size_t first = 0;
      for (int py = 0; py < 2; ++py)
        for (int px = 0; px < 2; ++px) {
          const size_t ci = add_conv(P, "", 0, M.fus_up[i][py * 2 + px], up_src, 0, up, 0, ST_FUS + 3 * i, ST_FUS + 3 * i + 1, 2, 2,
                                     py, px, nullptr, true);
          if (py == 0 && px == 0) first = ci;
        }
      P.h_probs[first].group = 4;
      const double up_bytes = 4.0 * P.last_conv_bytes;
      Plan* pq = &P;
      const double fl = 2.0 * 16.0 * M.fus_up[i][0].cin_ref * nf * (double)Hs[i + 1] * Ws[i + 1];
      P.add_op(0, "fusion_up@L" + std::to_string(i), [pq, first](cudaStream_t st) {
        return launch_conv_tc(pq->d_probs + first, pq->h_probs[first], st);
      }, fl, up_bytes);
      P.ops.back().form = "tc";
      P.ops.back().passes = P.h_probs[first].passes;
    } else {
      for (int py = 0; py < 2; ++py)
        for (int px = 0; px < 2; ++px)
          add_conv(P, "fusion_up" + std::to_string(py * 2 + px) + "@L" + std::to_string(i),
                   4.0 * M.fus_up[i][0].cin_ref * nf, M.fus_up[i][py * 2 + px], up_src, 0, up, 0, ST_FUS + 3 * i,
                   ST_FUS + 3 * i + 1, 2, 2, py, px);
    }
    P.debug["out:fusion_up@L" + std::to_string(i)] = DebugTensor{true, up->hi, up->lo, up->pixels(), up->C, 0, nf};
    SplitBuf* f1 = P.split(1, hh, ww, cpad);
    SplitBuf* f2 = (fuse_rgb && i == 0) ? nullptr : P.split(1, hh, ww, cpad);
    add_conv(P, "fusion_conv1@L" + std::to_string(i), 9.0 * M.fus_c1[i].cin_ref * nf, M.fus_c1[i],
             {{batch_view(wf[i], 0), 0}, {batch_view(wf[i], 1), 0}, {side[i], 0}, {up, 0}}, 1, f1, 0, ST_FUS + 3 * i + 1,
             ST_FUS + 3 * i + 2);
    if (fuse_rgb && i == 0) {
      const size_t ci = add_conv(P, "fusion_conv2+rgb@L0", 9.0 * nf * nf + 64.0 * 3, M.fus_c2[i], {{f1, 0}}, 1, nullptr, 0,
                                 ST_FUS + 3 * i + 2, ST_NONE, 1, 1, 0, 0, nullptr, false, 2);
      ConvProblem& hp = P.h_probs[ci];
      if (hp.cout != 64 || hp.bn != 64) throw Error{FILM_ERR_UNSUPPORTED, "RGB-head epilogue expects a 64-channel N tile"};
      hp.head_w4 = M.rgb_w;
      hp.head_b4 = M.rgb_b;
      hp.head_v = P.xout;
      hp.crop_y = P.off_y;
      hp.crop_x = P.off_x;
      hp.crop_h = P.h;
      hp.crop_w = P.w;
      hp.crop_pitch = (int64_t)P.w * 3;
    } else {
      add_conv(P, "fusion_conv2@L" + std::to_string(i), 9.0 * nf * nf, M.fus_c2[i], {{f1, 0}}, 1, f2, 0, ST_FUS + 3 * i + 2,
               i > 0 ? ST_FUS + 3 * (i - 1) : ST_NONE);
    }
    if (i == kFusionLevels - 2) P.release(wf[i + 1]);
    else P.release(net);
    P.release(wf[i]);
    P.release(up);
    P.release(f1);
    net = f2;
    if (f2) P.debug["fusion_net/" + std::to_string(i)] = DebugTensor{true, f2->hi, f2->lo, (int64_t)hh * ww, f2->C, 0, nf};
    P.debug["fusion_up/" + std::to_string(i)] = DebugTensor{true, up->hi, up->lo, (int64_t)hh * ww, up->C, 0, nf};
  }
  {
    const float *rw = M.rgb_w, *rb = M.rgb_b;
    if (!fuse_rgb)
      P.add_op(2, "rgb_head", [=](cudaStream_t st) {
        return launch_rgb_head(net->hi, net->lo, net->C, pp->H, pp->W, rw, rb, pp->xout, (int64_t)pp->w * 3, pp->off_y,
                               pp->off_x, pp->h, pp->w, st);
      });
    P.debug["image"] = DebugTensor{false, P.xout, nullptr, (int64_t)h * w, 3, 0, 3};
    P.tok_end = P.new_token();
    P.signal_last(P.tok_end);
  }

  {
    double fe = 0, fl = 0, fu = 0;
    for (int i = 0; i < kLevels; ++i) {
      const int depth = (kLevels - i) < kSubLevels ? (kLevels - i) : kSubLevels;
      int cin = 3;
      for (int j = 0; j < depth; ++j) {
        const double c = kFilters << j;
        fe += (double)Hs[i + j] * Ws[i + j] * 9.0 * (cin * c + c * c);
        cin = (int)c;
      }
    }
    fe *= 2;
    for (int l = 0; l < kLevels; ++l) {
      const double nf = kFlowFilters[l < kSpecialized ? l : kSpecialized], cin = 2.0 * feat_channels(l);
      fl += (double)Hs[l] * Ws[l] * (9 * cin * nf + 18 * nf * nf + nf * nf / 2 + nf);
    }
    fl *= 2;
    for (int i = 0; i < kFusionLevels - 1; ++i) {
      const double nf = fusion_filters(i), a_c = 2.0 * (3 + feat_channels(i)) + 4;
      const double cc = (i == kFusionLevels - 2) ? 2.0 * (3 + feat_channels(i + 1)) + 4 : fusion_filters(i + 1);
      fu += (double)Hs[i] * Ws[i] * (4 * cc * nf + 9 * (a_c + nf) * nf + 9 * nf * nf);
    }
    fu += (double)Hs[0] * Ws[0] * 64 * 3;
    P.conv_flops = 2.0 * (fe + fl + fu);
  }

  if (P.reuse)
    for (auto& kv : P.debug)
      if (P.block_bytes.count((void*)kv.second.p0) ||
          kv.first.compare(0, 4, "feat") == 0 || kv.first.compare(0, 6, "warped") == 0 ||
          kv.first.compare(0, 11, "flow_warped") == 0 || kv.first.compare(0, 8, "flow_vup") == 0)
        kv.second.recycled = true;
  FILM_CUDA(cudaMalloc(&P.d_probs, P.h_probs.size() * sizeof(ConvProblem)));
  P.allocs.push_back(P.d_probs);
  FILM_CUDA(cudaMemcpy(P.d_probs, P.h_probs.data(), P.h_probs.size() * sizeof(ConvProblem), cudaMemcpyHostToDevice));
  return pl;
}

}

using namespace film;

struct film_handle {
  int device = 0;
  cudaStream_t stream = nullptr;
  cudaEvent_t ev[4] = {nullptr, nullptr, nullptr, nullptr};
  std::unique_ptr<Model> model;
  std::map<std::vector<int>, std::unique_ptr<Plan>> plans;
  Plan* last_plan = nullptr;
  std::string err;
  Options opt;
  bool dev_events_valid = false;
  cudaStream_t copy_stream = nullptr;
  float* stage_in[2] = {nullptr, nullptr};
  float* stage_out[2] = {nullptr, nullptr};
  size_t stage_bytes = 0;
  cudaEvent_t ev_in[2] = {nullptr, nullptr}, ev_done[2] = {nullptr, nullptr}, ev_free[2] = {nullptr, nullptr},
              ev_out[2] = {nullptr, nullptr};
  cudaStream_t lane_streams[Plan::kNumLanes] = {};
  std::vector<cudaEvent_t> token_events;
  cudaEvent_t fork_event = nullptr;
  uint8_t* u8_stage = nullptr;
  size_t u8_bytes = 0;
  float* overlap_stage = nullptr;
  size_t overlap_bytes = 0;
  int num_sms = 132;
  std::vector<cudaEvent_t> op_events;
  film_profile_t prof;
};

static std::string g_create_error;

static int fail(film_handle* h, const Error& e) noexcept {
  try {
    if (h) h->err = e.msg; else g_create_error = e.msg;
  } catch (...) {
  }
  return e.code;
}
#define FILM_CATCH_ALL(h)                                                                                     \
  catch (const Error& e) { return fail(h, e); }                                                               \
  catch (const std::bad_alloc&) { return fail(h, Error{FILM_ERR_CUDA, "out of host memory"}); }               \
  catch (const std::exception& e) { return fail(h, Error{FILM_ERR_CUDA, std::string("internal error: ") + e.what()}); } \
  catch (...) { return fail(h, Error{FILM_ERR_CUDA, "unknown internal error"}); }

static void enqueue_plan(film_handle* h, Plan* P, cudaStream_t origin) {
  if (!h->opt.use_lanes) {
    for (auto& op : P->ops) FILM_CUDA(op.fn(origin));
    return;
  }
  if (!h->fork_event) FILM_CUDA(cudaEventCreateWithFlags(&h->fork_event, cudaEventDisableTiming));
  for (int i = 1; i < Plan::kNumLanes; ++i)
    if (!h->lane_streams[i]) FILM_CUDA(cudaStreamCreateWithFlags(&h->lane_streams[i], cudaStreamNonBlocking));
  while ((int)h->token_events.size() < P->num_tokens) {
    cudaEvent_t e;
    FILM_CUDA(cudaEventCreateWithFlags(&e, cudaEventDisableTiming));
    h->token_events.push_back(e);
  }
  auto lane_stream = [&](int lane) { return lane == 0 ? origin : h->lane_streams[lane]; };
  FILM_CUDA(cudaEventRecord(h->fork_event, origin));
  bool forked[Plan::kNumLanes] = {true};
  for (auto& op : P->ops) {
    cudaStream_t st = lane_stream(op.lane);
    if (!forked[op.lane]) {
      FILM_CUDA(cudaStreamWaitEvent(st, h->fork_event, 0));
      forked[op.lane] = true;
    }
    for (int t : op.waits) FILM_CUDA(cudaStreamWaitEvent(st, h->token_events[t], 0));
    FILM_CUDA(op.fn(st));
    for (int t : op.signals) FILM_CUDA(cudaEventRecord(h->token_events[t], st));
  }
  if (P->tok_end >= 0) FILM_CUDA(cudaStreamWaitEvent(origin, h->token_events[P->tok_end], 0));
}

static void drop_plans(film_handle* h) {
  cudaStreamSynchronize(h->stream);
  cudaDeviceSynchronize();
  (void)cudaGetLastError();
  h->last_plan = nullptr;
  h->dev_events_valid = false;
  h->plans.clear();
}

static Plan* get_plan(film_handle* h, int hh, int ww, int align) {
  if (!h->opt.any_size) {
    int H, W, oy, ox;
    padded_size(hh, ww, align, H, W, oy, ox);
    if (H % 64 || W % 64)
      throw Error{FILM_ERR_UNSUPPORTED,
                  "padded frame size must be a multiple of 64 (2^(pyramid_levels-1)) in this engine; use align=64"};
  }
  std::vector<int> key = {hh, ww, align > 0 ? align : 0};
  for (const OptionRow& r : kOptions)
    if (r.plan_key) key.push_back(h->opt.*r.field);
  auto it = h->plans.find(key);
  if (it != h->plans.end()) return it->second.get();
  auto build = [&] { return build_plan(*h->model, hh, ww, align, h->opt, h->num_sms); };
  std::unique_ptr<Plan> p;
  try {
    p = build();
  } catch (const Error& e0) {
    if (e0.code != FILM_ERR_CUDA || h->plans.empty()) throw;
    drop_plans(h);
    p = build();
  }
  if (h->opt.use_graph) {
    cudaGraph_t g = nullptr;
    FILM_CUDA(cudaStreamBeginCapture(h->stream, cudaStreamCaptureModeThreadLocal));
    try {
      enqueue_plan(h, p.get(), h->stream);
    } catch (const Error& err) {
      cudaStreamEndCapture(h->stream, &g);
      if (g) cudaGraphDestroy(g);
      (void)cudaGetLastError();
      throw Error{FILM_ERR_CUDA, "kernel launch failed during capture: " + err.msg};
    }
    FILM_CUDA(cudaStreamEndCapture(h->stream, &g));
    FILM_CUDA(cudaGraphInstantiate(&p->graph, g, 0));
    cudaGraphDestroy(g);
  }
  Plan* raw = p.get();
  h->plans[key] = std::move(p);
  return raw;
}

static void run_plan(film_handle* h, Plan* P, cudaStream_t st) {
  if (P->graph && !h->opt.time_ops) {
    FILM_CUDA(cudaGraphLaunch(P->graph, st));
  } else {
    if (h->opt.time_ops && st == h->stream) {
      const size_t n = P->ops.size();
      while (h->op_events.size() < n + 1) {
        cudaEvent_t e;
        FILM_CUDA(cudaEventCreate(&e));
        h->op_events.push_back(e);
      }
      FILM_CUDA(cudaEventRecord(h->op_events[0], st));
      for (size_t i = 0; i < n; ++i) {
        FILM_CUDA(P->ops[i].fn(st));
        FILM_CUDA(cudaEventRecord(h->op_events[i + 1], st));
      }
      FILM_CUDA(cudaStreamSynchronize(st));
      P->op_ms.assign(n, 0.f);
      for (size_t i = 0; i < n; ++i) FILM_CUDA(cudaEventElapsedTime(&P->op_ms[i], h->op_events[i], h->op_events[i + 1]));
    } else {
      enqueue_plan(h, P, st);
    }
  }
  h->last_plan = P;
}

extern "C" {

const char* film_version(void) {
  return "film_b200 0.3 sm_90a split=" FILM_SPLIT_NAME
         " mma=wgmma.f32, per-stage precision plan: 3-pass (hi*hi+hi*lo+lo*hi) or 1-pass (hi*hi)";
}

int film_create(film_handle** out, const char* weights_path, int device_ordinal) {
  if (!out || !weights_path) {
    g_create_error = "null argument";
    return FILM_ERR_ARG;
  }
  *out = nullptr;
  film_handle* h = nullptr;
  try {
    int ndev = 0;
    if (cudaGetDeviceCount(&ndev) != cudaSuccess || ndev == 0)
      throw Error{FILM_ERR_CUDA, "no CUDA device: the FILM engine has no CPU fallback"};
    if (device_ordinal < 0 || device_ordinal >= ndev) throw Error{FILM_ERR_ARG, "bad device ordinal"};
    FILM_CUDA(cudaSetDevice(device_ordinal));
    cudaDeviceProp prop;
    FILM_CUDA(cudaGetDeviceProperties(&prop, device_ordinal));
    if (prop.major != 9 || prop.minor != 0)
      throw Error{FILM_ERR_CUDA, std::string("device is sm_") + std::to_string(prop.major * 10 + prop.minor) +
                                     ", this engine is sm_90a-only (wgmma/TMA)"};
    h = new film_handle;
    h->device = device_ordinal;
    memset(&h->prof, 0, sizeof(h->prof));
    FILM_CUDA(cudaStreamCreateWithFlags(&h->stream, cudaStreamNonBlocking));
    for (auto& e : h->ev) FILM_CUDA(cudaEventCreate(&e));
    FILM_CUDA(conv_tc_configure());
    FILM_CUDA(conv3x3_tc_configure());
    for (const OptionRow& r : kOptions)
      if (const char* e = r.env ? getenv(r.env) : nullptr)
        h->opt.*r.field = r.normalise(r.field == &Options::onepass_mask ? (int)strtoul(e, nullptr, 0) : atoi(e));
    h->num_sms = prop.multiProcessorCount;
    WeightMap w = read_weight_file(weights_path);
    h->model.reset(new Model);
    h->model->load(w);
    *out = h;
    return FILM_OK;
  } catch (const Error& e) {
    fail(nullptr, e);
    if (h) film_destroy(h);
    return e.code;
  } catch (const std::exception& e) {
    fail(nullptr, Error{FILM_ERR_CUDA, std::string("internal error: ") + e.what()});
    if (h) film_destroy(h);
    return FILM_ERR_CUDA;
  } catch (...) {
    fail(nullptr, Error{FILM_ERR_CUDA, "unknown internal error"});
    if (h) film_destroy(h);
    return FILM_ERR_CUDA;
  }
}

void film_destroy(film_handle* h) {
  if (!h) return;
  cudaSetDevice(h->device);
  if (h->stream) cudaStreamSynchronize(h->stream);
  h->plans.clear();
  h->model.reset();
  for (auto& e : h->ev)
    if (e) cudaEventDestroy(e);
  for (auto& e : h->op_events) cudaEventDestroy(e);
  for (auto& e : h->token_events) cudaEventDestroy(e);
  for (int i = 0; i < 2; ++i) {
    if (h->stage_in[i]) cudaFree(h->stage_in[i]);
    if (h->stage_out[i]) cudaFree(h->stage_out[i]);
    for (cudaEvent_t e : {h->ev_in[i], h->ev_done[i], h->ev_free[i], h->ev_out[i]})
      if (e) cudaEventDestroy(e);
  }
  if (h->u8_stage) cudaFree(h->u8_stage);
  if (h->overlap_stage) cudaFree(h->overlap_stage);
  if (h->copy_stream) cudaStreamDestroy(h->copy_stream);
  if (h->fork_event) cudaEventDestroy(h->fork_event);
  for (int i = 1; i < Plan::kNumLanes; ++i)
    if (h->lane_streams[i]) cudaStreamDestroy(h->lane_streams[i]);
  if (h->stream) cudaStreamDestroy(h->stream);
  delete h;
}

const char* film_last_error(film_handle* h) { return h ? h->err.c_str() : g_create_error.c_str(); }

int film_set_option(film_handle* h, const char* name, int value) {
  if (!h || !name) return FILM_ERR_ARG;
  try {
    if (!strcmp(name, "onepass_default")) h->opt.onepass_mask = (int)kDefaultOnepassMask;
    else if (!strcmp(name, "clear_plans")) drop_plans(h);
    else {
      const OptionRow& r = option_row(name);
      h->opt.*r.field = r.normalise(value);
    }
    return FILM_OK;
  }
  FILM_CATCH_ALL(h)
}

int film_stage_count(void) { return ST_COUNT; }

int film_stage_name(int stage, char* buf, int buf_size) {
  if (!buf || buf_size < 1 || stage < 0 || stage >= ST_COUNT) return FILM_ERR_ARG;
  try {
    const std::string n = stage_name(stage);
    snprintf(buf, (size_t)buf_size, "%s", n.c_str());
    return FILM_OK;
  } catch (...) {
    return FILM_ERR_CUDA;
  }
}

int film_get_option(film_handle* h, const char* name, int* value) {
  if (!h || !name || !value) return FILM_ERR_ARG;
  try {
    *value = !strcmp(name, "onepass_default") ? (int)kDefaultOnepassMask : h->opt.*option_row(name).field;
    return FILM_OK;
  }
  FILM_CATCH_ALL(h)
}

int film_synchronize(film_handle* h) {
  if (!h) return FILM_ERR_ARG;
  try {
    FILM_CUDA(cudaSetDevice(h->device));
    FILM_CUDA(cudaStreamSynchronize(h->stream));
    return FILM_OK;
  }
  FILM_CATCH_ALL(h)
}

extern "C++" {
static void ensure_staging(film_handle* h, size_t frame_bytes) {
  if (!h->copy_stream) FILM_CUDA(cudaStreamCreateWithFlags(&h->copy_stream, cudaStreamNonBlocking));
  for (int i = 0; i < 2; ++i) {
    if (!h->ev_in[i]) {
      FILM_CUDA(cudaEventCreateWithFlags(&h->ev_in[i], cudaEventDisableTiming));
      FILM_CUDA(cudaEventCreateWithFlags(&h->ev_done[i], cudaEventDisableTiming));
      FILM_CUDA(cudaEventCreateWithFlags(&h->ev_free[i], cudaEventDisableTiming));
      FILM_CUDA(cudaEventCreateWithFlags(&h->ev_out[i], cudaEventDisableTiming));
    }
  }
  if (h->stage_bytes >= frame_bytes) return;
  for (int i = 0; i < 2; ++i) {
    if (h->stage_in[i]) cudaFree(h->stage_in[i]);
    if (h->stage_out[i]) cudaFree(h->stage_out[i]);
    h->stage_in[i] = h->stage_out[i] = nullptr;
  }
  h->stage_bytes = 0;
  for (int i = 0; i < 2; ++i) {
    FILM_CUDA(cudaMalloc(&h->stage_in[i], 2 * frame_bytes));
    FILM_CUDA(cudaMalloc(&h->stage_out[i], frame_bytes));
  }
  h->stage_bytes = frame_bytes;
}

template <class Fetch, class Deliver>
static void run_pipelined(film_handle* h, Plan* P, int n, size_t frame_bytes, Fetch fetch, Deliver deliver) {
  ensure_staging(h, frame_bytes);
  cudaStream_t cs = h->copy_stream, ms = h->stream;
  FILM_CUDA(cudaStreamSynchronize(ms));
  FILM_CUDA(cudaStreamSynchronize(cs));
  for (int i = 0; i < n; ++i) {
    const int b = i & 1;
    if (i >= 2) FILM_CUDA(cudaStreamWaitEvent(cs, h->ev_free[b], 0));
    fetch(i, h->stage_in[b], (float*)((char*)h->stage_in[b] + frame_bytes), cs);
    FILM_CUDA(cudaEventRecord(h->ev_in[b], cs));
    FILM_CUDA(cudaStreamWaitEvent(ms, h->ev_in[b], 0));
    FILM_CUDA(cudaMemcpyAsync(P->xin, h->stage_in[b], 2 * frame_bytes, cudaMemcpyDeviceToDevice, ms));
    FILM_CUDA(cudaEventRecord(h->ev_free[b], ms));
    run_plan(h, P, ms);
    if (i >= 2) FILM_CUDA(cudaStreamWaitEvent(ms, h->ev_out[b], 0));
    FILM_CUDA(cudaMemcpyAsync(h->stage_out[b], P->xout, frame_bytes, cudaMemcpyDeviceToDevice, ms));
    FILM_CUDA(cudaEventRecord(h->ev_done[b], ms));
    if (i >= 1) {
      const int pb = (i - 1) & 1;
      FILM_CUDA(cudaStreamWaitEvent(cs, h->ev_done[pb], 0));
      deliver(i - 1, h->stage_out[pb], cs);
      FILM_CUDA(cudaEventRecord(h->ev_out[pb], cs));
    }
  }
  const int lb = (n - 1) & 1;
  FILM_CUDA(cudaStreamWaitEvent(cs, h->ev_done[lb], 0));
  deliver(n - 1, h->stage_out[lb], cs);
  FILM_CUDA(cudaStreamSynchronize(cs));
  FILM_CUDA(cudaStreamSynchronize(ms));
}

}

static void check_frame_args(const void* x0, const void* x1, const void* out, int B, int H, int W) {
  if (!x0 || !x1 || !out) throw Error{FILM_ERR_ARG, "null frame pointer"};
  if (B < 1 || H < 1 || W < 1) throw Error{FILM_ERR_ARG, "batch, height and width must be positive"};
}

static void fill_profile(film_handle* h, Plan* P, float ms_net, float ms_h2d, float ms_d2h) {
  film_profile_t& p = h->prof;
  p.last_call_ms = ms_net;
  p.last_h2d_ms = ms_h2d;
  p.last_d2h_ms = ms_d2h;
  p.conv_flops = P->conv_flops;
  p.mma_flops = P->mma_flops;
  p.warp_bytes = P->warp_bytes;
  p.kernel_launches = (int64_t)P->ops.size();
  p.arena_bytes = P->arena_bytes;
  p.padded_h = P->H;
  p.padded_w = P->W;
  p.used_graph = P->graph ? 1 : 0;
}

int film_interpolate(film_handle* h, const float* x0, const float* x1, const float* dt, int B, int H, int W,
                     int align, float* out) {
  if (!h) return FILM_ERR_ARG;
  (void)dt;
  try {
    check_frame_args(x0, x1, out, B, H, W);
    FILM_CUDA(cudaSetDevice(h->device));
    (void)cudaGetLastError();
    Plan* P = get_plan(h, H, W, align);
    const size_t frame = (size_t)H * W * 3 * sizeof(float);
    float ms_net = 0, ms_h2d = 0, ms_d2h = 0;
    if (B > 1 && !h->opt.time_ops) {
      run_pipelined(h, P, B, frame,
                    [&](int b, float* d0, float* d1, cudaStream_t cs) {
                      FILM_CUDA(cudaMemcpyAsync(d0, (const char*)x0 + b * frame, frame, cudaMemcpyHostToDevice, cs));
                      FILM_CUDA(cudaMemcpyAsync(d1, (const char*)x1 + b * frame, frame, cudaMemcpyHostToDevice, cs));
                    },
                    [&](int b, const float* src, cudaStream_t cs) {
                      FILM_CUDA(cudaMemcpyAsync((char*)out + b * frame, src, frame, cudaMemcpyDeviceToHost, cs));
                    });
      fill_profile(h, P, 0.f, 0.f, 0.f);
      return FILM_OK;
    }
    for (int b = 0; b < B; ++b) {
      FILM_CUDA(cudaEventRecord(h->ev[0], h->stream));
      FILM_CUDA(cudaMemcpyAsync(P->xin, (const char*)x0 + b * frame, frame, cudaMemcpyHostToDevice, h->stream));
      FILM_CUDA(cudaMemcpyAsync((char*)P->xin + frame, (const char*)x1 + b * frame, frame, cudaMemcpyHostToDevice, h->stream));
      FILM_CUDA(cudaEventRecord(h->ev[1], h->stream));
      run_plan(h, P, h->stream);
      FILM_CUDA(cudaEventRecord(h->ev[2], h->stream));
      FILM_CUDA(cudaMemcpyAsync((char*)out + b * frame, P->xout, frame, cudaMemcpyDeviceToHost, h->stream));
      FILM_CUDA(cudaEventRecord(h->ev[3], h->stream));
      FILM_CUDA(cudaStreamSynchronize(h->stream));
      float t;
      FILM_CUDA(cudaEventElapsedTime(&t, h->ev[0], h->ev[1]));
      ms_h2d += t;
      FILM_CUDA(cudaEventElapsedTime(&t, h->ev[1], h->ev[2]));
      ms_net += t;
      FILM_CUDA(cudaEventElapsedTime(&t, h->ev[2], h->ev[3]));
      ms_d2h += t;
    }
    fill_profile(h, P, ms_net, ms_h2d, ms_d2h);
    return FILM_OK;
  }
  FILM_CATCH_ALL(h)
}

static void run_on_views(film_handle* h, Plan* P, const float* d_x0, const float* d_x1, int H, int W, int64_t in_pitch,
                         float* d_out, int64_t out_pitch, cudaStream_t st) {
  const size_t row = (size_t)W * 3 * sizeof(float);
  FILM_CUDA(cudaMemcpy2DAsync(P->xin, row, d_x0, in_pitch * 4, row, H, cudaMemcpyDeviceToDevice, st));
  FILM_CUDA(cudaMemcpy2DAsync(P->xin + (int64_t)H * W * 3, row, d_x1, in_pitch * 4, row, H, cudaMemcpyDeviceToDevice, st));
  FILM_CUDA(cudaEventRecord(h->ev[1], st));
  run_plan(h, P, st);
  FILM_CUDA(cudaEventRecord(h->ev[2], st));
  FILM_CUDA(cudaMemcpy2DAsync(d_out, out_pitch * 4, P->xout, row, row, H, cudaMemcpyDeviceToDevice, st));
}

int film_interpolate_device(film_handle* h, const float* d_x0, const float* d_x1, int B, int H, int W,
                            int64_t in_pitch, int align, float* d_out, int64_t out_pitch, void* cuda_stream) {
  if (!h) return FILM_ERR_ARG;
  try {
    check_frame_args(d_x0, d_x1, d_out, B, H, W);
    if (in_pitch < (int64_t)W * 3 || out_pitch < (int64_t)W * 3) throw Error{FILM_ERR_ARG, "pitch smaller than a row"};
    FILM_CUDA(cudaSetDevice(h->device));
    (void)cudaGetLastError();
    Plan* P = get_plan(h, H, W, align);
    cudaStream_t st = cuda_stream ? (cudaStream_t)cuda_stream : h->stream;
    for (int b = 0; b < B; ++b)
      run_on_views(h, P, d_x0 + (int64_t)b * H * in_pitch, d_x1 + (int64_t)b * H * in_pitch, H, W, in_pitch,
                   d_out + (int64_t)b * H * out_pitch, out_pitch, st);
    fill_profile(h, P, -1.f, 0.f, 0.f);
    h->dev_events_valid = true;
    return FILM_OK;
  }
  FILM_CATCH_ALL(h)
}

static StitchAxis stitch_axis(const char* name, int L, int b, int overlap) {
// ... 377 lines not shown
```

### frame_interpolation_b200/csrc/film_kernels.cu

```cuda
#include "film_conv.h"
#include "film_kernels.h"

namespace film {

static inline int cdiv(int64_t a, int64_t b) { return (int)((a + b - 1) / b); }

__device__ __forceinline__ uint4 ldg16(const void* p) { return __ldg(reinterpret_cast<const uint4*>(p)); }

__global__ void k_image_pool(const float* __restrict__ in, float* __restrict__ out, int B, int H,
                             int W) {
  const int Ho = H / 2, Wo = W / 2;
  const int64_t n = (int64_t)B * Ho * Wo * 3;
  int64_t i = (int64_t)blockIdx.x * blockDim.x + threadIdx.x;
  if (i >= n) return;
  int c = (int)(i % 3);
  int64_t p = i / 3;
  int x = (int)(p % Wo);
  p /= Wo;
  int y = (int)(p % Ho);
  int b = (int)(p / Ho);
  const float* r0 = in + (((int64_t)b * H + 2 * y) * W + 2 * x) * 3 + c;
  const float* r1 = r0 + (int64_t)W * 3;
  out[i] = (r0[0] + r0[3] + r1[0] + r1[3]) * 0.25f;
}

cudaError_t launch_image_pool(const float* in, float* out, int B, int H, int W, cudaStream_t st) {
  int64_t n = (int64_t)B * (H / 2) * (W / 2) * 3;
  if (n == 0) return cudaSuccess;
  k_image_pool<<<cdiv(n, 256), 256, 0, st>>>(in, out, B, H, W);
  return cudaGetLastError();
}

__global__ void k_pad_image(const float* __restrict__ src, int64_t src_pitch, int h, int w,
                            float* __restrict__ dst, int H, int W, int off_y, int off_x) {
  const int64_t n = (int64_t)H * W * 3;
  int64_t i = (int64_t)blockIdx.x * blockDim.x + threadIdx.x;
  if (i >= n) return;
  int c = (int)(i % 3);
  int64_t p = i / 3;
  int x = (int)(p % W), y = (int)(p / W);
  int sy = y - off_y, sx = x - off_x;
  float v = 0.f;
  if (sy >= 0 && sy < h && sx >= 0 && sx < w) v = src[(int64_t)sy * src_pitch + sx * 3 + c];
  dst[i] = v;
}

cudaError_t launch_pad_image(const float* src, int64_t src_pitch, int h, int w, float* dst, int H,
                             int W, int off_y, int off_x, cudaStream_t st) {
  int64_t n = (int64_t)H * W * 3;
  k_pad_image<<<cdiv(n, 256), 256, 0, st>>>(src, src_pitch, h, w, dst, H, W, off_y, off_x);
  return cudaGetLastError();
}

template <bool kVec>
__global__ void __launch_bounds__(256) k_u8_to_f32(const uint8_t* __restrict__ src, float* __restrict__ dst, int64_t n) {
  const int64_t i = ((int64_t)blockIdx.x * blockDim.x + threadIdx.x) * 4;
  if (kVec && i + 3 < n) {
    const uchar4 u = *reinterpret_cast<const uchar4*>(src + i);
    float4 f;
    f.x = __fdiv_rn((float)u.x, 255.f);
    f.y = __fdiv_rn((float)u.y, 255.f);
    f.z = __fdiv_rn((float)u.z, 255.f);
    f.w = __fdiv_rn((float)u.w, 255.f);
    *reinterpret_cast<float4*>(dst + i) = f;
  } else {
    for (int64_t j = i; j < n && j < i + 4; ++j) dst[j] = __fdiv_rn((float)src[j], 255.f);
  }
}
__device__ __forceinline__ uint8_t quantize_u8(float x) {
  const float s = fminf(fmaxf(__fmul_rn(x, 255.f), 0.f), 255.f);
  return (uint8_t)__fadd_rn(s, 0.5f);
}
template <bool kVec>
__global__ void __launch_bounds__(256) k_f32_to_u8(const float* __restrict__ src, uint8_t* __restrict__ dst, int64_t n) {
  const int64_t i = ((int64_t)blockIdx.x * blockDim.x + threadIdx.x) * 4;
  if (kVec && i + 3 < n) {
    const float4 f = *reinterpret_cast<const float4*>(src + i);
    uchar4 u;
    u.x = quantize_u8(f.x);
    u.y = quantize_u8(f.y);
    u.z = quantize_u8(f.z);
    u.w = quantize_u8(f.w);
    *reinterpret_cast<uchar4*>(dst + i) = u;
  } else {
    for (int64_t j = i; j < n && j < i + 4; ++j) dst[j] = quantize_u8(src[j]);
  }
}
cudaError_t launch_u8_to_f32(const uint8_t* src, float* dst, int64_t n, cudaStream_t st) {
  const bool vec = ((uintptr_t)src & 3) == 0 && ((uintptr_t)dst & 15) == 0;
  if (vec) k_u8_to_f32<true><<<cdiv(cdiv(n, 4), 256), 256, 0, st>>>(src, dst, n);
  else k_u8_to_f32<false><<<cdiv(cdiv(n, 4), 256), 256, 0, st>>>(src, dst, n);
  return cudaGetLastError();
}
cudaError_t launch_f32_to_u8(const float* src, uint8_t* dst, int64_t n, cudaStream_t st) {
  const bool vec = ((uintptr_t)src & 15) == 0 && ((uintptr_t)dst & 3) == 0;
  if (vec) k_f32_to_u8<true><<<cdiv(cdiv(n, 4), 256), 256, 0, st>>>(src, dst, n);
  else k_f32_to_u8<false><<<cdiv(cdiv(n, 4), 256), 256, 0, st>>>(src, dst, n);
  return cudaGetLastError();
}

__device__ __forceinline__ void stitch_sources(const StitchAxis& a, int x, int& ka, int& kb, float& t) {
  const int k = x / a.p, r = x - k * a.p;
  ka = kb = k;
  t = 0.f;
  if (k > 0 && r < a.v) {
    ka = k - 1;
    t = ((float)(r + a.v) + 0.5f) / (float)(2 * a.v);
  } else if (k < a.b - 1 && r >= a.p - a.v) {
    kb = k + 1;
    t = ((float)(r - (a.p - a.v)) + 0.5f) / (float)(2 * a.v);
  }
}

__device__ __forceinline__ void stitch_load(const float* __restrict__ p, int n, float (&v)[4]) {
  if (n == 4 && ((uintptr_t)p & 15) == 0) {
    const float4 f = __ldg(reinterpret_cast<const float4*>(p));
    v[0] = f.x, v[1] = f.y, v[2] = f.z, v[3] = f.w;
  } else {
#pragma unroll
    for (int i = 0; i < 4; ++i)
      if (i < n) v[i] = __ldg(p + i);
  }
}

__device__ __forceinline__ void stitch_run(const float* __restrict__ tiles, int64_t tile_stride, const StitchGeom& g, int y,
                                           int ya, int yb, float ty, int j, int n, float* __restrict__ o) {
  int xa = 0, xb = 0;
  float tx[4];
#pragma unroll
  for (int i = 0; i < 4; ++i)
    if (i < n) stitch_sources(g.ax, (j + i) / 3, xa, xb, tx[i]);
  auto src = [&](int ky, int kx) {
    return tiles + (int64_t)g.slot[ky * g.ax.b + kx] * tile_stride +
           ((int64_t)(y - stitch_origin(g.ay, ky)) * g.ax.q - stitch_origin(g.ax, kx)) * 3 + j;
  };
  auto row = [&](int ky, float (&r)[4]) {
    stitch_load(src(ky, xa), n, r);
    if (xb != xa) {
      float b[4];
      stitch_load(src(ky, xb), n, b);
#pragma unroll
      for (int i = 0; i < 4; ++i)
        if (i < n) r[i] = r[i] + tx[i] * (b[i] - r[i]);
    }
  };
  float r[4];
  row(ya, r);
  if (yb != ya) {
    float s[4];
    row(yb, s);
#pragma unroll
    for (int i = 0; i < 4; ++i)
      if (i < n) r[i] = r[i] + ty * (s[i] - r[i]);
  }
  if (n == 4 && ((uintptr_t)o & 15) == 0) {
    *reinterpret_cast<float4*>(o) = make_float4(r[0], r[1], r[2], r[3]);
  } else {
#pragma unroll
    for (int i = 0; i < 4; ++i)
      if (i < n) o[i] = r[i];
  }
}

__global__ void __launch_bounds__(256) k_stitch_feather(const float* __restrict__ tiles, int64_t tile_stride,
                                                        const __grid_constant__ StitchGeom g, float* __restrict__ out,
                                                        int64_t out_pitch) {
  const int row_floats = g.ax.L * 3;
  const int j = (blockIdx.x * blockDim.x + threadIdx.x) * 4;
  const int y = blockIdx.y;
  if (j >= row_floats) return;
  const int n = min(4, row_floats - j);
  int ya, yb, xa0, xb0, xa1, xb1;
  float ty, t;
  stitch_sources(g.ay, y, ya, yb, ty);
  stitch_sources(g.ax, j / 3, xa0, xb0, t);
  stitch_sources(g.ax, (j + n - 1) / 3, xa1, xb1, t);
  float* o = out + (int64_t)y * out_pitch + j;
  if (xa0 == xa1 && xb0 == xb1) {
    stitch_run(tiles, tile_stride, g, y, ya, yb, ty, j, n, o);
  } else {
    for (int i = 0; i < n; ++i) stitch_run(tiles, tile_stride, g, y, ya, yb, ty, j + i, 1, o + i);
  }
}

cudaError_t launch_stitch_feather(const float* tiles, int64_t tile_stride, const StitchGeom& g, float* out,
                                  int64_t out_pitch, cudaStream_t st) {
  dim3 grid(cdiv((int64_t)g.ax.L * 3, 4 * 256), g.ay.L);
  k_stitch_feather<<<grid, 256, 0, st>>>(tiles, tile_stride, g, out, out_pitch);
  return cudaGetLastError();
}

__global__ void __launch_bounds__(256) k_conv0_c3(const float* __restrict__ img, int B, int H, int W,
                                                  const float* __restrict__ w,
                                                  const float* __restrict__ bias,
                                                  sp_t* __restrict__ out_hi, sp_t* __restrict__ out_lo,
                                                  int out_C, int out_c_off) {
  __shared__ float ws[27 * 64];
  __shared__ float bs[64];
  for (int i = threadIdx.x; i < 27 * 64; i += 256) ws[i] = w[i];
  if (threadIdx.x < 64) bs[threadIdx.x] = bias[threadIdx.x];
  __syncthreads();
  const int64_t npix = (int64_t)B * H * W;
  int64_t p = (int64_t)blockIdx.x * 32 + (threadIdx.x >> 3);
  if (p >= npix) return;
  const int g = threadIdx.x & 7;
  int x = (int)(p % W);
  int64_t q = p / W;
  int y = (int)(q % H);
  int b = (int)(q / H);
  float acc[8];
#pragma unroll
  for (int j = 0; j < 8; ++j) acc[j] = 0.f;
#pragma unroll
  for (int ky = 0; ky < 3; ++ky) {
    int yy = y + ky - 1;
    if (yy < 0 || yy >= H) continue;
#pragma unroll
    for (int kx = 0; kx < 3; ++kx) {
      int xx = x + kx - 1;
      if (xx < 0 || xx >= W) continue;
      const float* ip = img + (((int64_t)b * H + yy) * W + xx) * 3;
#pragma unroll
      for (int ci = 0; ci < 3; ++ci) {
        float v = __ldg(ip + ci);
        const float* wr = ws + ((ky * 3 + kx) * 3 + ci) * 64 + g * 8;
#pragma unroll
        for (int j = 0; j < 8; ++j) acc[j] = fmaf(v, wr[j], acc[j]);
      }
    }
  }
#pragma unroll
  for (int j = 0; j < 8; ++j) acc[j] = leaky(acc[j] + bs[g * 8 + j]);
  uint4 h, l;
  pack8(acc, h, l);
  int64_t o = p * out_C + out_c_off + g * 8;
  *reinterpret_cast<uint4*>(out_hi + o) = h;
  *reinterpret_cast<uint4*>(out_lo + o) = l;
}

constexpr int kC0H = 8, kC0W = 16;
constexpr int kC0Tiles = 4;
constexpr int kC0Patch = (kC0H + 2) * (kC0W + 2) * 3;
constexpr int kC0PatchRegs = (kC0Patch + 127) / 128;
__device__ __forceinline__ float fe_patch_load(const float* __restrict__ img, int b, int H, int W, int y0, int x0, int i) {
  const int c = i % 3, px = (i / 3) % (kC0W + 2), py = i / (3 * (kC0W + 2));
  const int yy = y0 + py - 1, xx = x0 + px - 1;
  return (i < kC0Patch && yy >= 0 && yy < H && xx >= 0 && xx < W) ? __ldg(img + (((int64_t)b * H + yy) * W + xx) * 3 + c) : 0.f;
}
__global__ void __launch_bounds__(128) k_fe_conv0(const float* __restrict__ img, int H, int W,
                                                  const float* __restrict__ w, const float* __restrict__ bias,
                                                  sp_t* __restrict__ out_hi, sp_t* __restrict__ out_lo, int lo_skip,
                                                  float* __restrict__ pool_out) {
  __shared__ float4 ws[27 * 16];
  __shared__ float bs[64];
  __shared__ float patch[kC0Patch];
  const int tid = threadIdx.x;
  const int b = blockIdx.z, y0 = blockIdx.y * kC0H, xb = blockIdx.x * (kC0W * kC0Tiles);
  for (int i = tid; i < 27 * 16; i += 128) ws[i] = __ldg(reinterpret_cast<const float4*>(w) + i);
  if (tid < 64) bs[tid] = bias[tid];
  float nxt[kC0PatchRegs];
#pragma unroll
  for (int j = 0; j < kC0PatchRegs; ++j) nxt[j] = fe_patch_load(img, b, H, W, y0, xb, tid + 128 * j);
  const int warp = tid >> 5, lane = tid & 31;
  const int r = lane >> 2, cx = (lane & 3) * 4;
  const int y = y0 + r;
#pragma unroll 1
  for (int tile = 0; tile < kC0Tiles; ++tile) {
    const int x0 = xb + tile * kC0W;
    if (x0 >= W) break;
    __syncthreads();
#pragma unroll
    for (int j = 0; j < kC0PatchRegs; ++j)
      if (tid + 128 * j < kC0Patch) patch[tid + 128 * j] = nxt[j];
    __syncthreads();
    if (pool_out != nullptr && tid < (kC0H / 2) * (kC0W / 2) * 3) {
      const int c = tid % 3, qx = (tid / 3) % (kC0W / 2), qy = tid / (3 * (kC0W / 2));
      const int oy = (y0 >> 1) + qy, ox = (x0 >> 1) + qx;
      if (oy < (H >> 1) && ox < (W >> 1)) {
        const float* p0 = patch + ((2 * qy + 1) * (kC0W + 2) + 2 * qx + 1) * 3 + c;
        const float* p1 = p0 + (kC0W + 2) * 3;
        pool_out[(((int64_t)b * (H >> 1) + oy) * (W >> 1) + ox) * 3 + c] = (p0[0] + p0[3] + p1[0] + p1[3]) * 0.25f;
      }
    }
    if (tile + 1 < kC0Tiles && x0 + kC0W < W) {
#pragma unroll
      for (int j = 0; j < kC0PatchRegs; ++j) nxt[j] = fe_patch_load(img, b, H, W, y0, x0 + kC0W, tid + 128 * j);
    }
    float acc[4][16];
#pragma unroll
    for (int p = 0; p < 4; ++p)
#pragma unroll
      for (int j = 0; j < 16; ++j) acc[p][j] = 0.f;
#pragma unroll
    for (int ky = 0; ky < 3; ++ky) {
      float in[18];
      const float* pr = patch + ((r + ky) * (kC0W + 2) + cx) * 3;
#pragma unroll
      for (int j = 0; j < 18; ++j) in[j] = pr[j];
#pragma unroll
      for (int kx = 0; kx < 3; ++kx)
#pragma unroll
        for (int ci = 0; ci < 3; ++ci) {
          const float4* wk = ws + ((ky * 3 + kx) * 3 + ci) * 16 + warp * 4;
          const float4 w0 = wk[0], w1 = wk[1], w2 = wk[2], w3 = wk[3];
          const float wv[16] = {w0.x, w0.y, w0.z, w0.w, w1.x, w1.y, w1.z, w1.w, w2.x, w2.y, w2.z, w2.w, w3.x, w3.y, w3.z, w3.w};
#pragma unroll
          for (int p = 0; p < 4; ++p) {
            const float v = in[(p + kx) * 3 + ci];
#pragma unroll
            for (int j = 0; j < 16; ++j) acc[p][j] = fmaf(v, wv[j], acc[p][j]);
          }
        }
    }
    if (y < H) {
#pragma unroll
      for (int p = 0; p < 4; ++p) {
        const int x = x0 + cx + p;
        if (x < W) {
          float f[16];
#pragma unroll
          for (int j = 0; j < 16; ++j) f[j] = leaky(acc[p][j] + bs[warp * 16 + j]);
          const int64_t o = (((int64_t)b * H + y) * W + x) * 64 + warp * 16;
          if (lo_skip) pack_store16_hi(f, out_hi + o);
          else pack_store16(f, out_hi + o, out_lo + o);
        }
      }
    }
  }
}
cudaError_t launch_fe_conv0(const float* img, int B, int H, int W, const float* w, const float* bias, sp_t* out_hi,
                            sp_t* out_lo, bool lo_skip, float* pool_out, cudaStream_t st) {
  dim3 grid((W + kC0W * kC0Tiles - 1) / (kC0W * kC0Tiles), (H + kC0H - 1) / kC0H, B);
  k_fe_conv0<<<grid, 128, 0, st>>>(img, H, W, w, bias, out_hi, out_lo, lo_skip ? 1 : 0, pool_out);
  return cudaGetLastError();
}

cudaError_t launch_conv0_c3(const float* img, int B, int H, int W, const float* w,
                            const float* bias, sp_t* out_hi, sp_t* out_lo, int out_C,
                            int out_c_off, cudaStream_t st) {
  int64_t npix = (int64_t)B * H * W;
  k_conv0_c3<<<cdiv(npix, 32), 256, 0, st>>>(img, B, H, W, w, bias, out_hi, out_lo, out_C, out_c_off);
  return cudaGetLastError();
}

__global__ void __launch_bounds__(256) k_im2col3x3(const float* __restrict__ img, int B, int H, int W,
                                                   sp_t* __restrict__ out_hi, sp_t* __restrict__ out_lo) {
  const int64_t n = (int64_t)B * H * W * 4;
  int64_t i = (int64_t)blockIdx.x * blockDim.x + threadIdx.x;
  if (i >= n) return;
  const int g = (int)(i & 3);
  const int64_t p = i >> 2;
  const int x = (int)(p % W);
  const int64_t q = p / W;
  const int y = (int)(q % H);
  const int b = (int)(q / H);
  float v[8];
#pragma unroll
  for (int j = 0; j < 8; ++j) {
    const int k = g * 8 + j;
    float val = 0.f;
    if (k < 27) {
      const int tap = k / 3, ci = k - tap * 3;
      const int yy = y + tap / 3 - 1, xx = x + tap % 3 - 1;
      if (yy >= 0 && yy < H && xx >= 0 && xx < W) val = __ldg(img + (((int64_t)b * H + yy) * W + xx) * 3 + ci);
    }
    v[j] = val;
  }
  uint4 h, l;
  pack8(v, h, l);
  *reinterpret_cast<uint4*>(out_hi + p * 32 + g * 8) = h;
  *reinterpret_cast<uint4*>(out_lo + p * 32 + g * 8) = l;
}

__global__ void __launch_bounds__(256) k_image_to_split32(const float* __restrict__ img, int64_t npix,
                                                          sp_t* __restrict__ out_hi, sp_t* __restrict__ out_lo) {
  int64_t p = (int64_t)blockIdx.x * blockDim.x + threadIdx.x;
  if (p >= npix) return;
  float v[8] = {__ldg(img + p * 3), __ldg(img + p * 3 + 1), __ldg(img + p * 3 + 2), 0.f, 0.f, 0.f, 0.f, 0.f};
  uint4 h, l;
  pack8(v, h, l);
  *reinterpret_cast<uint4*>(out_hi + p * 32) = h;
  *reinterpret_cast<uint4*>(out_lo + p * 32) = l;
}

cudaError_t launch_image_to_split32(const float* img, int B, int H, int W, sp_t* out_hi, sp_t* out_lo, cudaStream_t st) {
  int64_t npix = (int64_t)B * H * W;
  k_image_to_split32<<<cdiv(npix, 256), 256, 0, st>>>(img, npix, out_hi, out_lo);
  return cudaGetLastError();
}

cudaError_t launch_im2col3x3(const float* img, int B, int H, int W, sp_t* out_hi, sp_t* out_lo, cudaStream_t st) {
  int64_t n = (int64_t)B * H * W * 4;
  k_im2col3x3<<<cdiv(n, 256), 256, 0, st>>>(img, B, H, W, out_hi, out_lo);
  return cudaGetLastError();
}

__global__ void k_act_pool(const sp_t* __restrict__ in_hi, const sp_t* __restrict__ in_lo, int in_C,
                           int in_c_off, int B, int H, int W, int Cn, sp_t* __restrict__ out_hi,
                           sp_t* __restrict__ out_lo, int out_C) {
  const int Ho = H / 2, Wo = W / 2, G = Cn / 8;
  const int64_t n = (int64_t)B * Ho * Wo * G;
  int64_t i = (int64_t)blockIdx.x * blockDim.x + threadIdx.x;
  if (i >= n) return;
  int g = (int)(i % G);
  int64_t p = i / G;
  int x = (int)(p % Wo);
  int64_t q = p / Wo;
  int y = (int)(q % Ho);
  int b = (int)(q / Ho);
  int64_t base = (((int64_t)b * H + 2 * y) * W + 2 * x) * in_C + in_c_off + g * 8;
  float a[8], t[8];
  unpack8(ldg16(in_hi + base), ldg16(in_lo + base), a);
  unpack8(ldg16(in_hi + base + in_C), ldg16(in_lo + base + in_C), t);
#pragma unroll
  for (int j = 0; j < 8; ++j) a[j] += t[j];
  base += (int64_t)W * in_C;
  unpack8(ldg16(in_hi + base), ldg16(in_lo + base), t);
#pragma unroll
  for (int j = 0; j < 8; ++j) a[j] += t[j];
  unpack8(ldg16(in_hi + base + in_C), ldg16(in_lo + base + in_C), t);
#pragma unroll
  for (int j = 0; j < 8; ++j) a[j] = (a[j] + t[j]) * 0.25f;
  uint4 h, l;
  pack8(a, h, l);
  int64_t o = p * out_C + g * 8;
  *reinterpret_cast<uint4*>(out_hi + o) = h;
  *reinterpret_cast<uint4*>(out_lo + o) = l;
}

cudaError_t launch_act_pool(const sp_t* in_hi, const sp_t* in_lo, int in_C, int in_c_off, int B,
                            int H, int W, int Cn, sp_t* out_hi, sp_t* out_lo, int out_C,
                            cudaStream_t st) {
  int64_t n = (int64_t)B * (H / 2) * (W / 2) * (Cn / 8);
  if (n == 0) return cudaSuccess;
  k_act_pool<<<cdiv(n, 256), 256, 0, st>>>(in_hi, in_lo, in_C, in_c_off, B, H, W, Cn, out_hi, out_lo,
                                          out_C);
  return cudaGetLastError();
}

struct ResizeTap {
  int lo, hi;
  float w;
};
__device__ __forceinline__ ResizeTap resize_tap(int dst, int in_size, float scale) {
  float src = ((float)dst + 0.5f) * scale - 0.5f;
  float fl = floorf(src);
  ResizeTap t;
  t.lo = max((int)fl, 0);
  t.hi = min((int)ceilf(src), in_size - 1);
  t.w = src - fl;
  return t;
}

__device__ __forceinline__ float2 upsampled_flow(const float* __restrict__ v_prev, int d, int Hc,
                                                 int Wc, int H, int W, int y, int x) {
  const float sy = (float)Hc / (float)H, sx = (float)Wc / (float)W;
  ResizeTap ty = resize_tap(y, Hc, sy), tx = resize_tap(x, Wc, sx);
  const float2* base = reinterpret_cast<const float2*>(v_prev) + (int64_t)d * Hc * Wc;
  float2 tl = __ldg(base + (int64_t)ty.lo * Wc + tx.lo), tr = __ldg(base + (int64_t)ty.lo * Wc + tx.hi);
  float2 bl = __ldg(base + (int64_t)ty.hi * Wc + tx.lo), br = __ldg(base + (int64_t)ty.hi * Wc + tx.hi);
  float2 r;
  {
    float a = 2.f * tl.x, b = 2.f * tr.x, c = 2.f * bl.x, e = 2.f * br.x;
    float top = a + (b - a) * tx.w, bot = c + (e - c) * tx.w;
    r.x = top + (bot - top) * ty.w;
  }
  {
    float a = 2.f * tl.y, b = 2.f * tr.y, c = 2.f * bl.y, e = 2.f * br.y;
    float top = a + (b - a) * tx.w, bot = c + (e - c) * tx.w;
    r.y = top + (bot - top) * ty.w;
  }
  return r;
}

struct WarpTap {
  int y0, x0;
  float ay, ax;
};
__device__ __forceinline__ WarpTap warp_tap(int y, int x, float fx, float fy, int H, int W) {
  float qy = (float)y + fy, qx = (float)x + fx;
  float fy0 = fminf(fmaxf(floorf(qy), 0.f), (float)(H - 2));
  float fx0 = fminf(fmaxf(floorf(qx), 0.f), (float)(W - 2));
  WarpTap t;
  t.y0 = (int)fy0;
  t.x0 = (int)fx0;
  t.ay = fminf(fmaxf(qy - fy0, 0.f), 1.f);
  t.ax = fminf(fmaxf(qx - fx0, 0.f), 1.f);
  return t;
}

__device__ __forceinline__ float lerp4(float tl, float tr, float bl, float br, float ax, float ay) {
  float top = ax * (tr - tl) + tl;
  float bot = ax * (br - bl) + bl;
  return ay * (bot - top) + top;
}

__device__ __forceinline__ void gather8(const sp_t* __restrict__ hi, const sp_t* __restrict__ lo,
                                        int W, int C, int c, const WarpTap& t, float* out) {
  const int64_t o00 = ((int64_t)t.y0 * W + t.x0) * C + c;
  const sp_t* h0 = hi + o00;
  const sp_t* l0 = lo + o00;
  const int row = W * C;
  float tl[8], tr[8], bl[8], br[8];
  unpack8(ldg16(h0), ldg16(l0), tl);
  unpack8(ldg16(h0 + C), ldg16(l0 + C), tr);
  unpack8(ldg16(h0 + row), ldg16(l0 + row), bl);
  unpack8(ldg16(h0 + row + C), ldg16(l0 + row + C), br);
#pragma unroll
  for (int j = 0; j < 8; ++j) out[j] = lerp4(tl[j], tr[j], bl[j], br[j], t.ax, t.ay);
}

__device__ __forceinline__ void gather16(const sp_t* __restrict__ hi, const sp_t* __restrict__ lo,
                                         int W, int C, int c, const WarpTap& t, float* out) {
  const int64_t o00 = ((int64_t)t.y0 * W + t.x0) * C + c;
  const sp_t* h0 = hi + o00;
  const sp_t* l0 = lo + o00;
  const int row = W * C;
  float a[16], b[16], top[16];
  load_unpack16(h0, l0, a);
  load_unpack16(h0 + C, l0 + C, b);
#pragma unroll
  for (int j = 0; j < 16; ++j) top[j] = t.ax * (b[j] - a[j]) + a[j];
  load_unpack16(h0 + row, l0 + row, a);
  load_unpack16(h0 + row + C, l0 + row + C, b);
#pragma unroll
  for (int j = 0; j < 16; ++j) {
    const float bot = t.ax * (b[j] - a[j]) + a[j];
    out[j] = t.ay * (bot - top[j]) + top[j];
  }
}

__device__ __forceinline__ void gather16_hi(const sp_t* __restrict__ hi, int W, int C, int c, const WarpTap& t,
                                            float* out) {
  const sp_t* h0 = hi + ((int64_t)t.y0 * W + t.x0) * C + c;
  const int row = W * C;
  float a[16], b[16], top[16];
  load_unpack16_hi(h0, a);
  load_unpack16_hi(h0 + C, b);
#pragma unroll
  for (int j = 0; j < 16; ++j) top[j] = t.ax * (b[j] - a[j]) + a[j];
  load_unpack16_hi(h0 + row, a);
  load_unpack16_hi(h0 + row + C, b);
#pragma unroll
  for (int j = 0; j < 16; ++j) {
    const float bot = t.ax * (b[j] - a[j]) + a[j];
    out[j] = t.ay * (bot - top[j]) + top[j];
  }
}

template <bool kHiOnly>
__global__ void __launch_bounds__(256) k_flow_warp(const float* __restrict__ v_prev, int Hc, int Wc,
                                                   const sp_t* __restrict__ feat_hi,
                                                   const sp_t* __restrict__ feat_lo, int H, int W, int C,
                                                   float* __restrict__ v_up, sp_t* __restrict__ warped_hi,
                                                   sp_t* __restrict__ warped_lo) {
  const int nchunk = C >> 6;
  const int d = blockIdx.z / nchunk;
  const int c = (blockIdx.z - d * nchunk) * 64 + (threadIdx.x & 3) * 16;
  const int x = blockIdx.x * 8 + ((threadIdx.x >> 2) & 7), y = blockIdx.y * 8 + (threadIdx.x >> 5);
  const int64_t p = ((int64_t)d * H + y) * W + x;
  __shared__ float2 sflow[64];
  const int pix = threadIdx.x >> 2;
  if ((threadIdx.x & 3) == 0 && x < W && y < H) sflow[pix] = upsampled_flow(v_prev, d, Hc, Wc, H, W, y, x);
  __syncthreads();
  if (x >= W || y >= H) return;
  const float2 f = sflow[pix];
  if (c == 0) reinterpret_cast<float2*>(v_up)[p] = f;
  WarpTap t = warp_tap(y, x, f.x, f.y, H, W);
  const int64_t src_off = (int64_t)(1 - d) * H * W * C;
  float o[16];
  if constexpr (kHiOnly) {
    gather16_hi(feat_hi + src_off, W, C, c, t, o);
    pack_store16_hi(o, warped_hi + p * C + c);
  } else {
    gather16(feat_hi + src_off, feat_lo + src_off, W, C, c, t, o);
    pack_store16(o, warped_hi + p * C + c, warped_lo + p * C + c);
  }
}

cudaError_t launch_flow_warp(const float* v_prev, int Hc, int Wc, const sp_t* feat_hi,
                             const sp_t* feat_lo, int H, int W, int C, float* v_up,
                             sp_t* warped_hi, sp_t* warped_lo, bool hi_only, cudaStream_t st) {
  dim3 grid((W + 7) / 8, (H + 7) / 8, 2 * (C / 64));
  if (hi_only) k_flow_warp<true><<<grid, 256, 0, st>>>(v_prev, Hc, Wc, feat_hi, feat_lo, H, W, C, v_up, warped_hi, warped_lo);
  else k_flow_warp<false><<<grid, 256, 0, st>>>(v_prev, Hc, Wc, feat_hi, feat_lo, H, W, C, v_up, warped_hi, warped_lo);
  return cudaGetLastError();
}

template <bool kHiOnly>
__global__ void __launch_bounds__(256) k_fusion_warp(const float* __restrict__ v,
                                                     const sp_t* __restrict__ feat_hi,
                                                     const sp_t* __restrict__ feat_lo, int H, int W,
                                                     int C, sp_t* __restrict__ warped_hi,
                                                     sp_t* __restrict__ warped_lo) {
  const int nchunk = C >> 6;
  const int k = blockIdx.z / nchunk;
  const int c = (blockIdx.z - k * nchunk) * 64 + (threadIdx.x & 3) * 16;
  const int x = blockIdx.x * 8 + ((threadIdx.x >> 2) & 7), y = blockIdx.y * 8 + (threadIdx.x >> 5);
  if (x >= W || y >= H) return;
  const int64_t p = ((int64_t)k * H + y) * W + x;
  float2 f = __ldg(reinterpret_cast<const float2*>(v) + ((int64_t)(1 - k) * H + y) * W + x);
  WarpTap t = warp_tap(y, x, f.x * 0.5f, f.y * 0.5f, H, W);
  const int64_t src_off = (int64_t)k * H * W * C;
  float o[16];
  if constexpr (kHiOnly) {
    gather16_hi(feat_hi + src_off, W, C, c, t, o);
    pack_store16_hi(o, warped_hi + p * C + c);
  } else {
    gather16(feat_hi + src_off, feat_lo + src_off, W, C, c, t, o);
    pack_store16(o, warped_hi + p * C + c, warped_lo + p * C + c);
  }
}

cudaError_t launch_fusion_warp(const float* v, const sp_t* feat_hi, const sp_t* feat_lo, int H,
                               int W, int C, sp_t* warped_hi, sp_t* warped_lo, bool hi_only, cudaStream_t st) {
  dim3 grid((W + 7) / 8, (H + 7) / 8, 2 * (C / 64));
  if (hi_only) k_fusion_warp<true><<<grid, 256, 0, st>>>(v, feat_hi, feat_lo, H, W, C, warped_hi, warped_lo);
  else k_fusion_warp<false><<<grid, 256, 0, st>>>(v, feat_hi, feat_lo, H, W, C, warped_hi, warped_lo);
  return cudaGetLastError();
}

__device__ __forceinline__ int nearest_src(int dst, int in, int out) {
  return min((int)(((int64_t)(2 * dst + 1) * in) / (2 * out)), in - 1);
}

template <bool kHiOnly>
__global__ void __launch_bounds__(256) k_resize_nearest(const sp_t* __restrict__ src_hi, const sp_t* __restrict__ src_lo,
                                                        int src_C, int src_c_off, int Hi, int Wi,
                                                        sp_t* __restrict__ dst_hi, sp_t* __restrict__ dst_lo, int dst_C,
                                                        int dst_c_off, int Ho, int Wo, int nvec, int64_t n) {
  const int64_t i = (int64_t)blockIdx.x * blockDim.x + threadIdx.x;
  if (i >= n) return;
  const int v = (int)(i % nvec);
  const int64_t p = i / nvec;
  const int x = (int)(p % Wo);
  const int64_t by = p / Wo;
  const int y = (int)(by % Ho), b = (int)(by / Ho);
  const int64_t sp = ((int64_t)b * Hi + nearest_src(y, Hi, Ho)) * Wi + nearest_src(x, Wi, Wo);
  const int64_t so = sp * src_C + src_c_off + 8 * v, d = p * dst_C + dst_c_off + 8 * v;
  *reinterpret_cast<uint4*>(dst_hi + d) = ldg16(src_hi + so);
  if constexpr (!kHiOnly) *reinterpret_cast<uint4*>(dst_lo + d) = ldg16(src_lo + so);
}

cudaError_t launch_resize_nearest(const sp_t* src_hi, const sp_t* src_lo, int src_C, int src_c_off, int B, int Hi, int Wi,
                                  sp_t* dst_hi, sp_t* dst_lo, int dst_C, int dst_c_off, int Ho, int Wo, int Cn, bool hi_only,
                                  cudaStream_t st) {
  if (Cn % 8 || src_C % 8 || dst_C % 8 || src_c_off % 8 || dst_c_off % 8) return cudaErrorInvalidValue;
  const int nvec = Cn / 8;
  const int64_t n = (int64_t)B * Ho * Wo * nvec;
  if (hi_only)
    k_resize_nearest<true><<<cdiv(n, 256), 256, 0, st>>>(src_hi, src_lo, src_C, src_c_off, Hi, Wi, dst_hi, dst_lo, dst_C,
                                                          dst_c_off, Ho, Wo, nvec, n);
  else
    k_resize_nearest<false><<<cdiv(n, 256), 256, 0, st>>>(src_hi, src_lo, src_C, src_c_off, Hi, Wi, dst_hi, dst_lo, dst_C,
                                                           dst_c_off, Ho, Wo, nvec, n);
  return cudaGetLastError();
}

__global__ void __launch_bounds__(256) k_fusion_side(const float* __restrict__ v,
                                                     const float* __restrict__ img, int H, int W,
                                                     sp_t* __restrict__ side_hi,
                                                     sp_t* __restrict__ side_lo, int side_C) {
  const int64_t n = (int64_t)H * W;
  int64_t p = (int64_t)blockIdx.x * blockDim.x + threadIdx.x;
  if (p >= n) return;
  int x = (int)(p % W), y = (int)(p / W);
  float o[16];
#pragma unroll
  for (int j = 0; j < 16; ++j) o[j] = 0.f;
#pragma unroll
  for (int k = 0; k < 2; ++k) {
    float2 f = __ldg(reinterpret_cast<const float2*>(v) + ((int64_t)(1 - k) * H + y) * W + x);
    f.x *= 0.5f;
    f.y *= 0.5f;
    WarpTap t = warp_tap(y, x, f.x, f.y, H, W);
    const float* ib = img + (int64_t)k * H * W * 3;
    const float* p00 = ib + ((int64_t)t.y0 * W + t.x0) * 3;
    const float* p10 = p00 + (int64_t)W * 3;
#pragma unroll
    for (int c = 0; c < 3; ++c)
      o[k * 3 + c] = lerp4(__ldg(p00 + c), __ldg(p00 + 3 + c), __ldg(p10 + c), __ldg(p10 + 3 + c), t.ax, t.ay);
    o[6 + 2 * k] = f.x;
    o[7 + 2 * k] = f.y;
  }
  uint4 h, l;
  pack8(o, h, l);
  int64_t oo = p * side_C;
  *reinterpret_cast<uint4*>(side_hi + oo) = h;
  *reinterpret_cast<uint4*>(side_lo + oo) = l;
  pack8(o + 8, h, l);
  *reinterpret_cast<uint4*>(side_hi + oo + 8) = h;
  *reinterpret_cast<uint4*>(side_lo + oo + 8) = l;
}

cudaError_t launch_fusion_side(const float* v, const float* img, int H, int W, sp_t* side_hi,
                               sp_t* side_lo, int side_C, cudaStream_t st) {
  int64_t n = (int64_t)H * W;
  k_fusion_side<<<cdiv(n, 256), 256, 0, st>>>(v, img, H, W, side_hi, side_lo, side_C);
  return cudaGetLastError();
}

constexpr int kHeadPix = 32;
__global__ void __launch_bounds__(128) k_flow_head(const sp_t* __restrict__ x_hi,
                                                   const sp_t* __restrict__ x_lo, int Cx, int nf,
                                                   int npix, const float* __restrict__ w3,
                                                   const float* __restrict__ b3,
                                                   const float* __restrict__ w4,
                                                   const float* __restrict__ b4,
                                                   const float* __restrict__ v_up,
                                                   float* __restrict__ residual, float* __restrict__ v) {
  extern __shared__ float smem[];
  const int J = nf / 2;
  float* xs = smem;
  float* hs = smem + kHeadPix * nf;
  const int64_t p0 = (int64_t)blockIdx.x * kHeadPix;
  const int G = nf / 8;
  for (int i = threadIdx.x; i < kHeadPix * G; i += 128) {
    int pp = i / G, g = i % G;
    float t[8];
    if (p0 + pp < npix) {
      int64_t o = (p0 + pp) * Cx + g * 8;
      unpack8(ldg16(x_hi + o), ldg16(x_lo + o), t);
    } else {
#pragma unroll
      for (int j = 0; j < 8; ++j) t[j] = 0.f;
    }
#pragma unroll
    for (int j = 0; j < 8; ++j) xs[pp * nf + g * 8 + j] = t[j];
  }
  __syncthreads();
  {
    const int j = threadIdx.x % J;
    const int groups = 128 / J > 0 ? 128 / J : 1;
    const int pg = threadIdx.x / J;
    if (pg < groups) {
      for (int pp = pg; pp < kHeadPix; pp += groups) {
        float acc = 0.f;
        const float* xr = xs + pp * nf;
        for (int k = 0; k < nf; ++k) acc = fmaf(xr[k], __ldg(w3 + k * J + j), acc);
        hs[pp * J + j] = leaky(acc + __ldg(b3 + j));
      }
    }
  }
  __syncthreads();
  if (threadIdx.x < kHeadPix * 2) {
    int pp = threadIdx.x >> 1, o = threadIdx.x & 1;
    if (p0 + pp < npix) {
      float acc = 0.f;
      const float* hr = hs + pp * J;
      for (int j = 0; j < J; ++j) acc = fmaf(hr[j], __ldg(w4 + j * 2 + o), acc);
      acc += __ldg(b4 + o);
      int64_t idx = (p0 + pp) * 2 + o;
      residual[idx] = acc;
      v[idx] = v_up ? acc + v_up[idx] : acc;
    }
  }
}

cudaError_t launch_flow_head(const sp_t* x_hi, const sp_t* x_lo, int Cx, int nf, int npix,
                             const float* w3, const float* b3, const float* w4, const float* b4,
                             const float* v_up, float* residual, float* v, cudaStream_t st) {
  size_t smem = (size_t)kHeadPix * (nf + nf / 2) * sizeof(float);
  k_flow_head<<<cdiv(npix, kHeadPix), 128, smem, st>>>(x_hi, x_lo, Cx, nf, npix, w3, b3, w4, b4, v_up,
                                                     residual, v);
  return cudaGetLastError();
}

__global__ void __launch_bounds__(256) k_rgb_head(const sp_t* __restrict__ x_hi,
                                                  const sp_t* __restrict__ x_lo, int Cx, int H, int W,
                                                  const float* __restrict__ w, const float* __restrict__ b,
                                                  float* __restrict__ out, int64_t out_pitch, int off_y,
                                                  int off_x, int out_h, int out_w) {
  __shared__ float ws[64 * 3 + 3];
  if (threadIdx.x < 64 * 3) ws[threadIdx.x] = w[threadIdx.x];
  if (threadIdx.x < 3) ws[192 + threadIdx.x] = b[threadIdx.x];
  __syncthreads();
  int64_t i = (int64_t)blockIdx.x * blockDim.x + threadIdx.x;
  if (i >= (int64_t)out_h * out_w) return;
  int ox = (int)(i % out_w), oy = (int)(i / out_w);
  int64_t p = (int64_t)(oy + off_y) * W + (ox + off_x);
  float a0 = 0.f, a1 = 0.f, a2 = 0.f;
#pragma unroll
  for (int g = 0; g < 8; ++g) {
    float t[8];
    unpack8(ldg16(x_hi + p * Cx + g * 8), ldg16(x_lo + p * Cx + g * 8), t);
#pragma unroll
    for (int j = 0; j < 8; ++j) {
      const float* wr = ws + (g * 8 + j) * 3;
      a0 = fmaf(t[j], wr[0], a0);
      a1 = fmaf(t[j], wr[1], a1);
      a2 = fmaf(t[j], wr[2], a2);
    }
  }
  float* o = out + (int64_t)oy * out_pitch + ox * 3;
  o[0] = a0 + ws[192];
  o[1] = a1 + ws[193];
  o[2] = a2 + ws[194];
}

cudaError_t launch_rgb_head(const sp_t* x_hi, const sp_t* x_lo, int Cx, int H, int W,
                            const float* w, const float* b, float* out, int64_t out_pitch,
                            int off_y, int off_x, int out_h, int out_w, cudaStream_t st) {
  int64_t n = (int64_t)out_h * out_w;
  k_rgb_head<<<cdiv(n, 256), 256, 0, st>>>(x_hi, x_lo, Cx, H, W, w, b, out, out_pitch, off_y, off_x,
                                          out_h, out_w);
  return cudaGetLastError();
}

__global__ void k_unsplit(const sp_t* __restrict__ hi, const sp_t* __restrict__ lo, int C, int c_off,
                          int Cn, int64_t npix, float* __restrict__ out) {
  int64_t i = (int64_t)blockIdx.x * blockDim.x + threadIdx.x;
  if (i >= npix * Cn) return;
  int c = (int)(i % Cn);
  int64_t p = i / Cn;
  int64_t o = p * C + c_off + c;
  out[i] = sp_to_float(hi[o]) + sp_to_float(lo[o]);
}

cudaError_t launch_unsplit(const sp_t* hi, const sp_t* lo, int C, int c_off, int Cn, int64_t npix,
                           float* out, cudaStream_t st) {
  int64_t n = npix * Cn;
  k_unsplit<<<cdiv(n, 256), 256, 0, st>>>(hi, lo, C, c_off, Cn, npix, out);
  return cudaGetLastError();
}

__global__ void __launch_bounds__(256) k_conv_simt(const ConvProblem* __restrict__ prob) {
  const ConvProblem& P = *prob;
  __shared__ float As[16][64 + 1];
  __shared__ float Ws[16][64 + 1];
  const int tid = threadIdx.x;
  const int tx = tid & 15, ty = tid >> 4;
  const int64_t npix = (int64_t)P.B * P.H * P.W;
  const int64_t m0 = (int64_t)blockIdx.x * 64;
  const int n0 = blockIdx.y * 64;
  float acc[4][4];
#pragma unroll
  for (int i = 0; i < 4; ++i)
#pragma unroll
    for (int j = 0; j < 4; ++j) acc[i][j] = 0.f;
  const int lm = tid >> 2, lk = (tid & 3) * 4;
  int64_t pm = m0 + lm;
  int px = 0, py = 0, pb = 0;
  const bool pm_ok = pm < npix;
  if (pm_ok) {
    px = (int)(pm % P.W);
    int64_t q = pm / P.W;
    py = (int)(q % P.H);
    pb = (int)(q / P.H);
  }
  int kb = 0;
  const int KC = P.kchunk;
  for (int s = 0; s < P.nsrc; ++s) {
    const ConvSrc& S = P.src[s];
    for (int ch = 0; ch < S.nchunk; ++ch) {
      for (int t = 0; t < P.ntaps; ++t, ++kb) {
        const int yy = py + P.tap_dy[t], xx = px + P.tap_dx[t];
        const bool ok = pm_ok && yy >= 0 && yy < P.H && xx >= 0 && xx < P.W;
        const int64_t abase = (((int64_t)(S.bswap ? P.B - 1 - pb : pb) * P.H + yy) * P.W + xx) * S.C + S.c_off + ch * KC;
        for (int k16 = 0; k16 < KC; k16 += 16) {
#pragma unroll
          for (int e = 0; e < 4; ++e) {
            float v = 0.f;
            if (ok) v = sp_to_float(S.hi[abase + k16 + lk + e]) + sp_to_float(S.lo[abase + k16 + lk + e]);
            As[lk + e][lm] = v;
          }
          {
            const int n = n0 + lm;
#pragma unroll
            for (int e = 0; e < 4; ++e) {
              float v = 0.f;
              if (n < P.cout) {
                int64_t wi = (int64_t)n * P.ktot + (int64_t)kb * KC + k16 + lk + e;
                v = sp_to_float(P.w_hi[wi]) + sp_to_float(P.w_lo[wi]);
              }
              Ws[lk + e][lm] = v;
            }
          }
          __syncthreads();
#pragma unroll
          for (int kk = 0; kk < 16; ++kk) {
            float a[4], b[4];
#pragma unroll
            for (int i = 0; i < 4; ++i) a[i] = As[kk][ty * 4 + i];
#pragma unroll
            for (int j = 0; j < 4; ++j) b[j] = Ws[kk][tx * 4 + j];
#pragma unroll
            for (int i = 0; i < 4; ++i)
#pragma unroll
              for (int j = 0; j < 4; ++j) acc[i][j] = fmaf(a[i], b[j], acc[i][j]);
          }
          __syncthreads();
        }
      }
    }
  }
#pragma unroll
  for (int i = 0; i < 4; ++i) {
    int64_t m = m0 + ty * 4 + i;
    if (m >= npix) continue;
    int x = (int)(m % P.W);
    int64_t q = m / P.W;
    int y = (int)(q % P.H);
    int b = (int)(q / P.H);
    int64_t opix = ((int64_t)b * P.out_H + (y * P.out_sy + P.out_oy)) * P.out_W + (x * P.out_sx + P.out_ox);
#pragma unroll
    for (int j = 0; j < 4; ++j) {
      int n = n0 + tx * 4 + j;
      if (n >= P.cout) continue;
      float v = acc[i][j] + P.bias[n];
      if (P.act) v = leaky(v);
      sp_t h, l;
      split2(v, h, l);
      int64_t o = opix * P.out_C + P.out_c_off + n;
      P.out_hi[o] = h;
      P.out_lo[o] = l;
    }
  }
}

cudaError_t launch_conv_simt(const ConvProblem* d_prob, const ConvProblem& h, cudaStream_t st) {
  int64_t npix = (int64_t)h.B * h.H * h.W;
  dim3 grid(cdiv(npix, 64), cdiv(h.cout, 64));
  k_conv_simt<<<grid, 256, 0, st>>>(d_prob);
  return cudaGetLastError();
}

}
```

Baseline: 26.54.

## Enable programmatic dependent launch across all kernels in the frame pipeline

Adds a launch helper that sets the programmatic stream serialization attribute, and inserts griddepcontrol wait/launch_dependents into every kernel. The next kernel's launch and prologue (barrier init, weight staging, setup) can then overlap the tail of the previous kernel, hiding launch gaps between many small kernels. Elementwise kernels trigger dependents immediately after waiting. The risk is correctness if any kernel touches dependent memory before its wait; in the 1x1 conv, warps above index 8 skip the wait, and producers trigger only after their loop.

Result: no change. 26.55, median of 6 (+0.0%).

```diff
diff --git a/frame_interpolation_b200/csrc/film_common.cuh b/frame_interpolation_b200/csrc/film_common.cuh
--- a/frame_interpolation_b200/csrc/film_common.cuh
+++ b/frame_interpolation_b200/csrc/film_common.cuh
@@ -165,4 +165,44 @@
 
 __device__ __forceinline__ float leaky(float x) { return x >= 0.f ? x : x * kLeaky; }
 
-}
+__device__ __forceinline__ void pdl_wait() { asm volatile("griddepcontrol.wait;" ::: "memory"); }
+__device__ __forceinline__ void pdl_trigger() { asm volatile("griddepcontrol.launch_dependents;" ::: "memory"); }
+
+inline bool& pdl_launches() {
+  static thread_local bool on = false;
+  return on;
+}
+struct PdlScope {
+  bool saved;
+  explicit PdlScope(bool on) : saved(pdl_launches()) { pdl_launches() = on; }
+  ~PdlScope() { pdl_launches() = saved; }
+};
+
+template <typename... KArgs, typename... Args>
+inline cudaError_t launch_kernel(void (*kernel)(KArgs...), dim3 grid, dim3 block, size_t smem, cudaStream_t st,
+                                 int cluster_x, Args&&... args) {
+  cudaLaunchAttribute attr[2];
+  unsigned n = 0;
+  if (cluster_x > 1) {
+    attr[n].id = cudaLaunchAttributeClusterDimension;
+    attr[n].val.clusterDim.x = cluster_x;
+    attr[n].val.clusterDim.y = 1;
+    attr[n].val.clusterDim.z = 1;
+    ++n;
+  }
+  if (pdl_launches()) {
+    attr[n].id = cudaLaunchAttributeProgrammaticStreamSerialization;
+    attr[n].val.programmaticStreamSerializationAllowed = 1;
+    ++n;
+  }
+  cudaLaunchConfig_t cfg = {};
+  cfg.gridDim = grid;
+  cfg.blockDim = block;
+  cfg.dynamicSmemBytes = smem;
+  cfg.stream = st;
+  cfg.attrs = attr;
+  cfg.numAttrs = n;
+  return cudaLaunchKernelEx(&cfg, kernel, static_cast<Args&&>(args)...);
+}
+
+}
diff --git a/frame_interpolation_b200/csrc/film_conv3x3_tc.cu b/frame_interpolation_b200/csrc/film_conv3x3_tc.cu
--- a/frame_interpolation_b200/csrc/film_conv3x3_tc.cu
+++ b/frame_interpolation_b200/csrc/film_conv3x3_tc.cu
@@ -128,6 +128,7 @@
       }
     }
     __syncwarp();
+    pdl_wait();
     RingPos ra, rw;
     for (int tile = w_first; tile < nwork; tile += w_step) {
       int sp, nti, b, rem, ty, tx;
@@ -202,6 +203,7 @@
         }
       }
     }
+    pdl_trigger();
     leave();
     return;
   }
@@ -240,6 +242,7 @@
   float* const head_res = prob->head_res;
   float* const head_vout = prob->head_v;
 
+  pdl_wait();
   if (resident) mbar_wait(tail + 8u * (2 * kMaxRing), 0);
   const bool is_leader = (threadIdx.x & 127) == 0;
   const uint32_t w_empty_peer = pair ? map_to_cta(tail + 8u * (3 * kMaxRing), (uint32_t)(rank ^ 1)) : 0u;
@@ -705,23 +708,7 @@
     if (kPxN && (h.pair || h.tile_h != 32 || h.tile_w != 8 || h.epi_mode != 0)) return cudaErrorInvalidValue;
     const bool partial = h.v2_part_hi > h.v2_part_lo;
     const int idx = (partial ? 8 : 0) | (h.halo ? 4 : 0) | (h.passes == 1 ? 2 : 0) | (h.v2_resident && h.straight ? 1 : 0);
-    if (!h.pair) {
-      kFn[idx]<<<h.v2_grid, kThreads, smem_bytes_for(h, BN), st>>>(d_prob);
-      return cudaGetLastError();
-    }
-    cudaLaunchConfig_t cfg = {};
-    cudaLaunchAttribute attr[1];
-    attr[0].id = cudaLaunchAttributeClusterDimension;
-    attr[0].val.clusterDim.x = 2;
-    attr[0].val.clusterDim.y = 1;
-    attr[0].val.clusterDim.z = 1;
-    cfg.gridDim = dim3(h.v2_grid);
-    cfg.blockDim = dim3(kThreads);
-    cfg.dynamicSmemBytes = smem_bytes_for(h, BN);
-    cfg.stream = st;
-    cfg.attrs = attr;
-    cfg.numAttrs = 1;
-    return cudaLaunchKernelEx(&cfg, kFn[idx], d_prob);
+    return launch_kernel(kFn[idx], h.v2_grid, kThreads, smem_bytes_for(h, BN), st, h.pair ? 2 : 1, d_prob);
   }
 };
 
diff --git a/frame_interpolation_b200/csrc/film_conv_tc.cu b/frame_interpolation_b200/csrc/film_conv_tc.cu
--- a/frame_interpolation_b200/csrc/film_conv_tc.cu
+++ b/frame_interpolation_b200/csrc/film_conv_tc.cu
@@ -73,6 +73,7 @@
     }
   }
   __syncthreads();
+  if (warp <= 8) pdl_wait();
 
   if (warp >= 8) {
     regs_dec<40>();
@@ -106,6 +107,7 @@
         }
       }
     }
+    pdl_trigger();
     return;
   }
 
@@ -220,8 +222,7 @@
 template <int BN, int KC>
 cudaError_t launch_bn(const ConvProblem* d_prob, const ConvProblem& h, cudaStream_t st) {
   dim3 grid(h.B * h.tiles_y * h.tiles_x, (h.cout + BN - 1) / BN, h.group > 1 ? h.group : 1);
-  k_conv_tc<BN, KC><<<grid, kNumThreads, TcCfg<BN, KC>::kSmemBytes, st>>>(d_prob);
-  return cudaGetLastError();
+  return launch_kernel(k_conv_tc<BN, KC>, grid, kNumThreads, TcCfg<BN, KC>::kSmemBytes, st, 1, d_prob);
 }
 
 }
diff --git a/frame_interpolation_b200/csrc/film_engine.cu b/frame_interpolation_b200/csrc/film_engine.cu
--- a/frame_interpolation_b200/csrc/film_engine.cu
+++ b/frame_interpolation_b200/csrc/film_engine.cu
@@ -79,6 +79,7 @@
   int arena_reuse = 1;
   int any_size = 0;
   int tile_overlap = 0;
+  int pdl = 1;
 };
 
 static int as_given(int v) { return v; }
@@ -112,6 +113,7 @@
     {"arena_reuse", &Options::arena_reuse, as_bool, "FILM_ARENA_REUSE", true},
     {"any_size", &Options::any_size, as_bool, nullptr, false},
     {"tile_overlap", &Options::tile_overlap, non_negative, nullptr, false},
+    {"pdl", &Options::pdl, as_bool, "FILM_PDL", true},
 };
 static const OptionRow& option_row(const char* name) {
   for (const OptionRow& r : kOptions)
@@ -1241,6 +1243,7 @@
   catch (...) { return fail(h, Error{FILM_ERR_CUDA, "unknown internal error"}); }
 
 static void enqueue_plan(film_handle* h, Plan* P, cudaStream_t origin) {
+  PdlScope pdl(P->opt.pdl != 0);
   if (!h->opt.use_lanes) {
     for (auto& op : P->ops) FILM_CUDA(op.fn(origin));
     return;
@@ -1331,6 +1334,7 @@
         FILM_CUDA(cudaEventCreate(&e));
         h->op_events.push_back(e);
       }
+      PdlScope pdl(P->opt.pdl != 0);
       FILM_CUDA(cudaEventRecord(h->op_events[0], st));
       for (size_t i = 0; i < n; ++i) {
         FILM_CUDA(P->ops[i].fn(st));
diff --git a/frame_interpolation_b200/csrc/film_kernels.cu b/frame_interpolation_b200/csrc/film_kernels.cu
--- a/frame_interpolation_b200/csrc/film_kernels.cu
+++ b/frame_interpolation_b200/csrc/film_kernels.cu
@@ -9,6 +9,8 @@
 
 __global__ void k_image_pool(const float* __restrict__ in, float* __restrict__ out, int B, int H,
                              int W) {
+  pdl_wait();
+  pdl_trigger();
   const int Ho = H / 2, Wo = W / 2;
   const int64_t n = (int64_t)B * Ho * Wo * 3;
   int64_t i = (int64_t)blockIdx.x * blockDim.x + threadIdx.x;
@@ -27,12 +29,13 @@
 cudaError_t launch_image_pool(const float* in, float* out, int B, int H, int W, cudaStream_t st) {
   int64_t n = (int64_t)B * (H / 2) * (W / 2) * 3;
   if (n == 0) return cudaSuccess;
-  k_image_pool<<<cdiv(n, 256), 256, 0, st>>>(in, out, B, H, W);
-  return cudaGetLastError();
+  return launch_kernel(k_image_pool, cdiv(n, 256), 256, 0, st, 1, in, out, B, H, W);
 }
 
 __global__ void k_pad_image(const float* __restrict__ src, int64_t src_pitch, int h, int w,
                             float* __restrict__ dst, int H, int W, int off_y, int off_x) {
+  pdl_wait();
+  pdl_trigger();
   const int64_t n = (int64_t)H * W * 3;
   int64_t i = (int64_t)blockIdx.x * blockDim.x + threadIdx.x;
   if (i >= n) return;
@@ -48,12 +51,13 @@
 cudaError_t launch_pad_image(const float* src, int64_t src_pitch, int h, int w, float* dst, int H,
                              int W, int off_y, int off_x, cudaStream_t st) {
   int64_t n = (int64_t)H * W * 3;
-  k_pad_image<<<cdiv(n, 256), 256, 0, st>>>(src, src_pitch, h, w, dst, H, W, off_y, off_x);
-  return cudaGetLastError();
+  return launch_kernel(k_pad_image, cdiv(n, 256), 256, 0, st, 1, src, src_pitch, h, w, dst, H, W, off_y, off_x);
 }
 
 template <bool kVec>
 __global__ void __launch_bounds__(256) k_u8_to_f32(const uint8_t* __restrict__ src, float* __restrict__ dst, int64_t n) {
+  pdl_wait();
+  pdl_trigger();
   const int64_t i = ((int64_t)blockIdx.x * blockDim.x + threadIdx.x) * 4;
   if (kVec && i + 3 < n) {
     const uchar4 u = *reinterpret_cast<const uchar4*>(src + i);
@@ -73,6 +77,8 @@
 }
 template <bool kVec>
 __global__ void __launch_bounds__(256) k_f32_to_u8(const float* __restrict__ src, uint8_t* __restrict__ dst, int64_t n) {
+  pdl_wait();
+  pdl_trigger();
   const int64_t i = ((int64_t)blockIdx.x * blockDim.x + threadIdx.x) * 4;
   if (kVec && i + 3 < n) {
     const float4 f = *reinterpret_cast<const float4*>(src + i);
@@ -88,15 +94,13 @@
 }
 cudaError_t launch_u8_to_f32(const uint8_t* src, float* dst, int64_t n, cudaStream_t st) {
   const bool vec = ((uintptr_t)src & 3) == 0 && ((uintptr_t)dst & 15) == 0;
-  if (vec) k_u8_to_f32<true><<<cdiv(cdiv(n, 4), 256), 256, 0, st>>>(src, dst, n);
-  else k_u8_to_f32<false><<<cdiv(cdiv(n, 4), 256), 256, 0, st>>>(src, dst, n);
-  return cudaGetLastError();
+  if (vec) return launch_kernel(k_u8_to_f32<true>, cdiv(cdiv(n, 4), 256), 256, 0, st, 1, src, dst, n);
+  else return launch_kernel(k_u8_to_f32<false>, cdiv(cdiv(n, 4), 256), 256, 0, st, 1, src, dst, n);
 }
 cudaError_t launch_f32_to_u8(const float* src, uint8_t* dst, int64_t n, cudaStream_t st) {
   const bool vec = ((uintptr_t)src & 15) == 0 && ((uintptr_t)dst & 3) == 0;
-  if (vec) k_f32_to_u8<true><<<cdiv(cdiv(n, 4), 256), 256, 0, st>>>(src, dst, n);
-  else k_f32_to_u8<false><<<cdiv(cdiv(n, 4), 256), 256, 0, st>>>(src, dst, n);
-  return cudaGetLastError();
+  if (vec) return launch_kernel(k_f32_to_u8<true>, cdiv(cdiv(n, 4), 256), 256, 0, st, 1, src, dst, n);
+  else return launch_kernel(k_f32_to_u8<false>, cdiv(cdiv(n, 4), 256), 256, 0, st, 1, src, dst, n);
 }
 
 __device__ __forceinline__ void stitch_sources(const StitchAxis& a, int x, int& ka, int& kb, float& t) {
@@ -165,6 +169,8 @@
 __global__ void __launch_bounds__(256) k_stitch_feather(const float* __restrict__ tiles, int64_t tile_stride,
                                                         const __grid_constant__ StitchGeom g, float* __restrict__ out,
                                                         int64_t out_pitch) {
+  pdl_wait();
+  pdl_trigger();
   const int row_floats = g.ax.L * 3;
   const int j = (blockIdx.x * blockDim.x + threadIdx.x) * 4;
   const int y = blockIdx.y;
@@ -186,8 +192,7 @@
 cudaError_t launch_stitch_feather(const float* tiles, int64_t tile_stride, const StitchGeom& g, float* out,
                                   int64_t out_pitch, cudaStream_t st) {
   dim3 grid(cdiv((int64_t)g.ax.L * 3, 4 * 256), g.ay.L);
-  k_stitch_feather<<<grid, 256, 0, st>>>(tiles, tile_stride, g, out, out_pitch);
-  return cudaGetLastError();
+  return launch_kernel(k_stitch_feather, grid, 256, 0, st, 1, tiles, tile_stride, g, out, out_pitch);
 }
 
 __global__ void __launch_bounds__(256) k_conv0_c3(const float* __restrict__ img, int B, int H, int W,
@@ -195,6 +200,8 @@
                                                   const float* __restrict__ bias,
                                                   sp_t* __restrict__ out_hi, sp_t* __restrict__ out_lo,
                                                   int out_C, int out_c_off) {
+  pdl_wait();
+  pdl_trigger();
   __shared__ float ws[27 * 64];
   __shared__ float bs[64];
   for (int i = threadIdx.x; i < 27 * 64; i += 256) ws[i] = w[i];
@@ -251,6 +258,8 @@
                                                   const float* __restrict__ w, const float* __restrict__ bias,
                                                   sp_t* __restrict__ out_hi, sp_t* __restrict__ out_lo, int lo_skip,
                                                   float* __restrict__ pool_out) {
+  pdl_wait();
+  pdl_trigger();
   __shared__ float4 ws[27 * 16];
   __shared__ float bs[64];
   __shared__ float patch[kC0Patch];
@@ -331,20 +340,20 @@
 cudaError_t launch_fe_conv0(const float* img, int B, int H, int W, const float* w, const float* bias, sp_t* out_hi,
                             sp_t* out_lo, bool lo_skip, float* pool_out, cudaStream_t st) {
   dim3 grid((W + kC0W * kC0Tiles - 1) / (kC0W * kC0Tiles), (H + kC0H - 1) / kC0H, B);
-  k_fe_conv0<<<grid, 128, 0, st>>>(img, H, W, w, bias, out_hi, out_lo, lo_skip ? 1 : 0, pool_out);
-  return cudaGetLastError();
+  return launch_kernel(k_fe_conv0, grid, 128, 0, st, 1, img, H, W, w, bias, out_hi, out_lo, lo_skip ? 1 : 0, pool_out);
 }
 
 cudaError_t launch_conv0_c3(const float* img, int B, int H, int W, const float* w,
                             const float* bias, sp_t* out_hi, sp_t* out_lo, int out_C,
                             int out_c_off, cudaStream_t st) {
   int64_t npix = (int64_t)B * H * W;
-  k_conv0_c3<<<cdiv(npix, 32), 256, 0, st>>>(img, B, H, W, w, bias, out_hi, out_lo, out_C, out_c_off);
-  return cudaGetLastError();
+  return launch_kernel(k_conv0_c3, cdiv(npix, 32), 256, 0, st, 1, img, B, H, W, w, bias, out_hi, out_lo, out_C, out_c_off);
 }
 
 __global__ void __launch_bounds__(256) k_im2col3x3(const float* __restrict__ img, int B, int H, int W,
                                                    sp_t* __restrict__ out_hi, sp_t* __restrict__ out_lo) {
+  pdl_wait();
+  pdl_trigger();
   const int64_t n = (int64_t)B * H * W * 4;
   int64_t i = (int64_t)blockIdx.x * blockDim.x + threadIdx.x;
   if (i >= n) return;
@@ -374,6 +383,8 @@
 
 __global__ void __launch_bounds__(256) k_image_to_split32(const float* __restrict__ img, int64_t npix,
                                                           sp_t* __restrict__ out_hi, sp_t* __restrict__ out_lo) {
+  pdl_wait();
+  pdl_trigger();
   int64_t p = (int64_t)blockIdx.x * blockDim.x + threadIdx.x;
   if (p >= npix) return;
   float v[8] = {__ldg(img + p * 3), __ldg(img + p * 3 + 1), __ldg(img + p * 3 + 2), 0.f, 0.f, 0.f, 0.f, 0.f};
@@ -385,19 +396,19 @@
 
 cudaError_t launch_image_to_split32(const float* img, int B, int H, int W, sp_t* out_hi, sp_t* out_lo, cudaStream_t st) {
   int64_t npix = (int64_t)B * H * W;
-  k_image_to_split32<<<cdiv(npix, 256), 256, 0, st>>>(img, npix, out_hi, out_lo);
-  return cudaGetLastError();
+  return launch_kernel(k_image_to_split32, cdiv(npix, 256), 256, 0, st, 1, img, npix, out_hi, out_lo);
 }
 
 cudaError_t launch_im2col3x3(const float* img, int B, int H, int W, sp_t* out_hi, sp_t* out_lo, cudaStream_t st) {
   int64_t n = (int64_t)B * H * W * 4;
-  k_im2col3x3<<<cdiv(n, 256), 256, 0, st>>>(img, B, H, W, out_hi, out_lo);
-  return cudaGetLastError();
+  return launch_kernel(k_im2col3x3, cdiv(n, 256), 256, 0, st, 1, img, B, H, W, out_hi, out_lo);
 }
 
 __global__ void k_act_pool(const sp_t* __restrict__ in_hi, const sp_t* __restrict__ in_lo, int in_C,
                            int in_c_off, int B, int H, int W, int Cn, sp_t* __restrict__ out_hi,
                            sp_t* __restrict__ out_lo, int out_C) {
+  pdl_wait();
+  pdl_trigger();
   const int Ho = H / 2, Wo = W / 2, G = Cn / 8;
   const int64_t n = (int64_t)B * Ho * Wo * G;
   int64_t i = (int64_t)blockIdx.x * blockDim.x + threadIdx.x;
@@ -433,9 +444,8 @@
                             cudaStream_t st) {
   int64_t n = (int64_t)B * (H / 2) * (W / 2) * (Cn / 8);
   if (n == 0) return cudaSuccess;
-  k_act_pool<<<cdiv(n, 256), 256, 0, st>>>(in_hi, in_lo, in_C, in_c_off, B, H, W, Cn, out_hi, out_lo,
+  return launch_kernel(k_act_pool, cdiv(n, 256), 256, 0, st, 1, in_hi, in_lo, in_C, in_c_off, B, H, W, Cn, out_hi, out_lo,
                                           out_C);
-  return cudaGetLastError();
 }
 
 struct ResizeTap {
@@ -554,6 +564,8 @@
                                                    const sp_t* __restrict__ feat_lo, int H, int W, int C,
                                                    float* __restrict__ v_up, sp_t* __restrict__ warped_hi,
                                                    sp_t* __restrict__ warped_lo) {
+  pdl_wait();
+  pdl_trigger();
   const int nchunk = C >> 6;
   const int d = blockIdx.z / nchunk;
   const int c = (blockIdx.z - d * nchunk) * 64 + (threadIdx.x & 3) * 16;
@@ -582,9 +594,8 @@
                              const sp_t* feat_lo, int H, int W, int C, float* v_up,
                              sp_t* warped_hi, sp_t* warped_lo, bool hi_only, cudaStream_t st) {
   dim3 grid((W + 7) / 8, (H + 7) / 8, 2 * (C / 64));
-  if (hi_only) k_flow_warp<true><<<grid, 256, 0, st>>>(v_prev, Hc, Wc, feat_hi, feat_lo, H, W, C, v_up, warped_hi, warped_lo);
-  else k_flow_warp<false><<<grid, 256, 0, st>>>(v_prev, Hc, Wc, feat_hi, feat_lo, H, W, C, v_up, warped_hi, warped_lo);
-  return cudaGetLastError();
+  if (hi_only) return launch_kernel(k_flow_warp<true>, grid, 256, 0, st, 1, v_prev, Hc, Wc, feat_hi, feat_lo, H, W, C, v_up, warped_hi, warped_lo);
+  else return launch_kernel(k_flow_warp<false>, grid, 256, 0, st, 1, v_prev, Hc, Wc, feat_hi, feat_lo, H, W, C, v_up, warped_hi, warped_lo);
 }
 
 template <bool kHiOnly>
@@ -593,6 +604,8 @@
                                                      const sp_t* __restrict__ feat_lo, int H, int W,
                                                      int C, sp_t* __restrict__ warped_hi,
                                                      sp_t* __restrict__ warped_lo) {
+  pdl_wait();
+  pdl_trigger();
   const int nchunk = C >> 6;
   const int k = blockIdx.z / nchunk;
   const int c = (blockIdx.z - k * nchunk) * 64 + (threadIdx.x & 3) * 16;
@@ -615,9 +628,8 @@
 cudaError_t launch_fusion_warp(const float* v, const sp_t* feat_hi, const sp_t* feat_lo, int H,
                                int W, int C, sp_t* warped_hi, sp_t* warped_lo, bool hi_only, cudaStream_t st) {
   dim3 grid((W + 7) / 8, (H + 7) / 8, 2 * (C / 64));
-  if (hi_only) k_fusion_warp<true><<<grid, 256, 0, st>>>(v, feat_hi, feat_lo, H, W, C, warped_hi, warped_lo);
-  else k_fusion_warp<false><<<grid, 256, 0, st>>>(v, feat_hi, feat_lo, H, W, C, warped_hi, warped_lo);
-  return cudaGetLastError();
+  if (hi_only) return launch_kernel(k_fusion_warp<true>, grid, 256, 0, st, 1, v, feat_hi, feat_lo, H, W, C, warped_hi, warped_lo);
+  else return launch_kernel(k_fusion_warp<false>, grid, 256, 0, st, 1, v, feat_hi, feat_lo, H, W, C, warped_hi, warped_lo);
 }
 
 __device__ __forceinline__ int nearest_src(int dst, int in, int out) {
@@ -629,6 +641,8 @@
                                                         int src_C, int src_c_off, int Hi, int Wi,
                                                         sp_t* __restrict__ dst_hi, sp_t* __restrict__ dst_lo, int dst_C,
                                                         int dst_c_off, int Ho, int Wo, int nvec, int64_t n) {
+  pdl_wait();
+  pdl_trigger();
   const int64_t i = (int64_t)blockIdx.x * blockDim.x + threadIdx.x;
   if (i >= n) return;
   const int v = (int)(i % nvec);
@@ -649,18 +663,19 @@
   const int nvec = Cn / 8;
   const int64_t n = (int64_t)B * Ho * Wo * nvec;
   if (hi_only)
-    k_resize_nearest<true><<<cdiv(n, 256), 256, 0, st>>>(src_hi, src_lo, src_C, src_c_off, Hi, Wi, dst_hi, dst_lo, dst_C,
+    return launch_kernel(k_resize_nearest<true>, cdiv(n, 256), 256, 0, st, 1, src_hi, src_lo, src_C, src_c_off, Hi, Wi, dst_hi, dst_lo, dst_C,
                                                           dst_c_off, Ho, Wo, nvec, n);
   else
-    k_resize_nearest<false><<<cdiv(n, 256), 256, 0, st>>>(src_hi, src_lo, src_C, src_c_off, Hi, Wi, dst_hi, dst_lo, dst_C,
+    return launch_kernel(k_resize_nearest<false>, cdiv(n, 256), 256, 0, st, 1, src_hi, src_lo, src_C, src_c_off, Hi, Wi, dst_hi, dst_lo, dst_C,
                                                            dst_c_off, Ho, Wo, nvec, n);
-  return cudaGetLastError();
 }
 
 __global__ void __launch_bounds__(256) k_fusion_side(const float* __restrict__ v,
                                                      const float* __restrict__ img, int H, int W,
                                                      sp_t* __restrict__ side_hi,
                                                      sp_t* __restrict__ side_lo, int side_C) {
+  pdl_wait();
+  pdl_trigger();
   const int64_t n = (int64_t)H * W;
   int64_t p = (int64_t)blockIdx.x * blockDim.x + threadIdx.x;
   if (p >= n) return;
@@ -696,8 +711,7 @@
 cudaError_t launch_fusion_side(const float* v, const float* img, int H, int W, sp_t* side_hi,
                                sp_t* side_lo, int side_C, cudaStream_t st) {
   int64_t n = (int64_t)H * W;
-  k_fusion_side<<<cdiv(n, 256), 256, 0, st>>>(v, img, H, W, side_hi, side_lo, side_C);
-  return cudaGetLastError();
+  return launch_kernel(k_fusion_side, cdiv(n, 256), 256, 0, st, 1, v, img, H, W, side_hi, side_lo, side_C);
 }
 
 constexpr int kHeadPix = 32;
@@ -709,6 +723,8 @@
                                                    const float* __restrict__ b4,
                                                    const float* __restrict__ v_up,
                                                    float* __restrict__ residual, float* __restrict__ v) {
+  pdl_wait();
+  pdl_trigger();
   extern __shared__ float smem[];
   const int J = nf / 2;
   float* xs = smem;
@@ -761,9 +777,8 @@
                              const float* w3, const float* b3, const float* w4, const float* b4,
                              const float* v_up, float* residual, float* v, cudaStream_t st) {
   size_t smem = (size_t)kHeadPix * (nf + nf / 2) * sizeof(float);
-  k_flow_head<<<cdiv(npix, kHeadPix), 128, smem, st>>>(x_hi, x_lo, Cx, nf, npix, w3, b3, w4, b4, v_up,
+  return launch_kernel(k_flow_head, cdiv(npix, kHeadPix), 128, smem, st, 1, x_hi, x_lo, Cx, nf, npix, w3, b3, w4, b4, v_up,
                                                      residual, v);
-  return cudaGetLastError();
 }
 
 __global__ void __launch_bounds__(256) k_rgb_head(const sp_t* __restrict__ x_hi,
@@ -771,6 +786,8 @@
                                                   const float* __restrict__ w, const float* __restrict__ b,
                                                   float* __restrict__ out, int64_t out_pitch, int off_y,
                                                   int off_x, int out_h, int out_w) {
+  pdl_wait();
+  pdl_trigger();
   __shared__ float ws[64 * 3 + 3];
   if (threadIdx.x < 64 * 3) ws[threadIdx.x] = w[threadIdx.x];
   if (threadIdx.x < 3) ws[192 + threadIdx.x] = b[threadIdx.x];
@@ -802,13 +819,14 @@
                             const float* w, const float* b, float* out, int64_t out_pitch,
                             int off_y, int off_x, int out_h, int out_w, cudaStream_t st) {
   int64_t n = (int64_t)out_h * out_w;
-  k_rgb_head<<<cdiv(n, 256), 256, 0, st>>>(x_hi, x_lo, Cx, H, W, w, b, out, out_pitch, off_y, off_x,
+  return launch_kernel(k_rgb_head, cdiv(n, 256), 256, 0, st, 1, x_hi, x_lo, Cx, H, W, w, b, out, out_pitch, off_y, off_x,
                                           out_h, out_w);
-  return cudaGetLastError();
 }
 
 __global__ void k_unsplit(const sp_t* __restrict__ hi, const sp_t* __restrict__ lo, int C, int c_off,
                           int Cn, int64_t npix, float* __restrict__ out) {
+  pdl_wait();
+  pdl_trigger();
   int64_t i = (int64_t)blockIdx.x * blockDim.x + threadIdx.x;
   if (i >= npix * Cn) return;
   int c = (int)(i % Cn);
@@ -820,11 +838,12 @@
 cudaError_t launch_unsplit(const sp_t* hi, const sp_t* lo, int C, int c_off, int Cn, int64_t npix,
                            float* out, cudaStream_t st) {
   int64_t n = npix * Cn;
-  k_unsplit<<<cdiv(n, 256), 256, 0, st>>>(hi, lo, C, c_off, Cn, npix, out);
-  return cudaGetLastError();
+  return launch_kernel(k_unsplit, cdiv(n, 256), 256, 0, st, 1, hi, lo, C, c_off, Cn, npix, out);
 }
 
 __global__ void __launch_bounds__(256) k_conv_simt(const ConvProblem* __restrict__ prob) {
+  pdl_wait();
+  pdl_trigger();
   const ConvProblem& P = *prob;
   __shared__ float As[16][64 + 1];
   __shared__ float Ws[16][64 + 1];
@@ -921,8 +940,7 @@
 cudaError_t launch_conv_simt(const ConvProblem* d_prob, const ConvProblem& h, cudaStream_t st) {
   int64_t npix = (int64_t)h.B * h.H * h.W;
   dim3 grid(cdiv(npix, 64), cdiv(h.cout, 64));
-  k_conv_simt<<<grid, 256, 0, st>>>(d_prob);
-  return cudaGetLastError();
-}
-
-}
+  return launch_kernel(k_conv_simt, grid, 256, 0, st, 1, d_prob);
+}
+
+}
```
